# uclanlp/visualbert

Measured on NVIDIA H100. Metric: image-text pairs/sec fwd+bwd VisualBERT-base, higher is better.
Workload: dtype bf16

## Files before the change

### visualbert_b200/csrc/vb_api.cu

```cuda
#include <string.h>

#include "vb_internal.h"

namespace vb {

constexpr float kLnEps = 1e-12f;
constexpr unsigned kEmbedDropStream = 0xE0000001u;
enum { kSiteAttnProbs = 0, kSiteAttnOut = 1, kSiteFfnOut = 2 };
static inline unsigned drop_stream(unsigned layer, unsigned site) { return layer * 8u + site; }

#define VB_TRY(expr)            \
    do {                        \
        int _rc = (expr);       \
        if (_rc) return _rc;    \
    } while (0)

static vb_gemm_args fwd_args(const void* A, const void* W, void* D, int M, int N, int K) {
    vb_gemm_args a;
    memset(&a, 0, sizeof(a));
    a.A = A; a.lda = K; a.B = W; a.ldb = K; a.M = M; a.N = N; a.K = K; a.D = D; a.ldd = N;
    return a;
}
static vb_gemm_args dgrad_args(const void* dY, const void* W, void* dX, int M, int N, int K) {
    vb_gemm_args a;
    memset(&a, 0, sizeof(a));
    a.A = dY; a.lda = N; a.B = W; a.ldb = K; a.b_mn_major = 1; a.M = M; a.N = K; a.K = N; a.D = dX; a.ldd = K;
    return a;
}
static vb_gemm_args wgrad_args(const void* dY, const void* X, float* dW, int M, int N, int K) {
    vb_gemm_args a;
    memset(&a, 0, sizeof(a));
    a.A = dY; a.lda = N; a.a_mn_major = 1; a.B = X; a.ldb = K; a.b_mn_major = 1;
    a.M = N; a.N = K; a.K = M; a.D = dW; a.ldd = K; a.d_fp32 = 1;
    return a;
}

struct LayerRows {
    const int* cu_seqlens;
    int total;
};
static const LayerRows kDenseRows = {nullptr, 0};

static int check_layer(const vb_layer_desc* d, const LayerRows& r) {
    VB_REQUIRE(d != nullptr, "layer: null descriptor");
    VB_REQUIRE(d->batch > 0 && d->seq > 0, "layer: empty batch");
    VB_REQUIRE(d->hidden == d->heads * 64, "layer: hidden (%d) must equal heads (%d) * 64", d->hidden, d->heads);
    VB_REQUIRE(d->hidden % 16 == 0 && d->inter % 16 == 0, "layer: hidden/intermediate must be multiples of 16");
    VB_REQUIRE(d->w_qkv && d->w_attn_out && d->w_inter && d->w_out, "layer: null weight pointer");
    VB_REQUIRE(r.cu_seqlens != nullptr || d->mask_bias != nullptr, "layer: null mask_bias");
    VB_REQUIRE(r.cu_seqlens == nullptr || r.total > 0, "layer: varlen call without rows (total = %d)", r.total);
    return 0;
}

int layer_fwd(const vb_layer_desc* d, const void* x_in, void* x_out, const vb_layer_acts* s, cudaStream_t st,
              const LayerRows& rows = kDenseRows, bool for_bwd = true) {
    VB_TRY(check_layer(d, rows));
    VB_REQUIRE(x_in && x_out && s, "layer_fwd: null pointer");
    const bool vl = rows.cu_seqlens != nullptr;
    const int M = vl ? rows.total : d->batch * d->seq, H = d->hidden, I = d->inter;
    vb_gemm_args a = fwd_args(x_in, d->w_qkv, s->qkv, M, 3 * H, H);
    a.bias = d->b_qkv;
    VB_TRY(gemm(a, st));
    if (vl)
        VB_TRY(attn_fwd_varlen(s->qkv, rows.cu_seqlens, s->ctx, s->lse, s->keep_mask, d->batch, d->seq, rows.total, d->heads, H,
                               d->attn_dropout, d->seed, drop_stream(d->layer_index, kSiteAttnProbs), st, for_bwd));
    else
        VB_TRY(attn_fwd(s->qkv, d->mask_bias, s->ctx, s->lse, s->keep_mask, d->batch, d->seq, d->heads, H, d->attn_dropout, d->seed,
                        drop_stream(d->layer_index, kSiteAttnProbs), st));
    a = fwd_args(s->ctx, d->w_attn_out, s->pre1, M, H, H);
    a.bias = d->b_attn_out; a.addend = x_in; a.ld_add = H;
    a.dropout_p = d->hidden_dropout; a.dropout_seed = d->seed; a.dropout_stream = drop_stream(d->layer_index, kSiteAttnOut);
    VB_TRY(gemm(a, st));
    VB_TRY(ln_fwd(s->pre1, H, d->ln1_gamma, d->ln1_beta, s->x1, H, s->mean1, s->rstd1, M, H, kLnEps, st));
    if (for_bwd) {
        a = fwd_args(s->x1, d->w_inter, s->u, M, I, H);
        a.bias = d->b_inter; a.epilogue = VB_EPI_GELU; a.aux_out = s->g; a.ld_aux = I;
        a.gp_tiled = gemm_gp_tiled_ok(M, I) ? 1 : 0;
    } else {
        a = fwd_args(s->x1, d->w_inter, s->g, M, I, H);
        a.bias = d->b_inter; a.epilogue = VB_EPI_GELU_FWD;
    }
    VB_TRY(gemm(a, st));
    a = fwd_args(s->g, d->w_out, s->pre2, M, H, I);
    a.bias = d->b_out; a.addend = s->x1; a.ld_add = H;
    a.dropout_p = d->hidden_dropout; a.dropout_seed = d->seed; a.dropout_stream = drop_stream(d->layer_index, kSiteFfnOut);
    VB_TRY(gemm(a, st));
    VB_TRY(ln_fwd(s->pre2, H, d->ln2_gamma, d->ln2_beta, x_out, H, s->mean2, s->rstd2, M, H, kLnEps, st));
    return 0;
}

static long long layer_bwd_det_bytes(int M, int H, int I) {
    const long long c = colsum_det_bytes(M, I) > colsum_det_bytes(M, 3 * H) ? colsum_det_bytes(M, I) : colsum_det_bytes(M, 3 * H);
    return ln_bwd_det_bytes(M, H) > c ? ln_bwd_det_bytes(M, H) : c;
}

int layer_bwd(const vb_layer_desc* d, const void* x_in, const vb_layer_acts* s, const void* dy, void* dx,
              const vb_layer_grads* g, const vb_layer_scratch* w, cudaStream_t st, const LayerRows& rows = kDenseRows) {
    VB_TRY(check_layer(d, rows));
    VB_REQUIRE(x_in && s && dy && dx && g && w, "layer_bwd: null pointer");
    const bool vl = rows.cu_seqlens != nullptr;
    const int M = vl ? rows.total : d->batch * d->seq, H = d->hidden, I = d->inter;
    VB_TRY(det_require(layer_bwd_det_bytes(M, H, I), "layer backward"));
    const bool hd = d->hidden_dropout > 0.f;
    VB_REQUIRE(!hd || w->d_pre_drop, "layer_bwd: d_pre_drop scratch required when hidden_dropout > 0");
    void* dpm = hd ? w->d_pre_drop : w->d_pre;

    VB_TRY(ln_bwd(dy, s->pre2, s->mean2, s->rstd2, d->ln2_gamma, w->d_pre, hd ? w->d_pre_drop : nullptr, g->dln2_gamma,
                  g->dln2_beta, g->db_out, M, H, d->hidden_dropout, d->seed, drop_stream(d->layer_index, kSiteFfnOut),
                  0.f, 0, st));
    VB_TRY(gemm(wgrad_args(dpm, s->g, g->dw_out, M, H, I), st));
    vb_gemm_args a = dgrad_args(dpm, d->w_out, w->d_big, M, H, I);
    a.epilogue = VB_EPI_DGELU; a.aux_in = s->u; a.ld_aux = I;
    a.gp_tiled = gemm_gp_tiled_ok(M, I) ? 1 : 0;
    VB_TRY(gemm(a, st));
    VB_TRY(colsum(w->d_big, I, g->db_inter, M, I, st));
    VB_TRY(gemm(wgrad_args(w->d_big, s->x1, g->dw_inter, M, I, H), st));
    a = dgrad_args(w->d_big, d->w_inter, w->d_x1, M, I, H);
    a.addend = w->d_pre; a.ld_add = H;
    VB_TRY(gemm(a, st));
    VB_TRY(ln_bwd(w->d_x1, s->pre1, s->mean1, s->rstd1, d->ln1_gamma, w->d_pre, hd ? w->d_pre_drop : nullptr,
                  g->dln1_gamma, g->dln1_beta, g->db_attn_out, M, H, d->hidden_dropout, d->seed,
                  drop_stream(d->layer_index, kSiteAttnOut), 0.f, 0, st));
    VB_TRY(gemm(wgrad_args(dpm, s->ctx, g->dw_attn_out, M, H, H), st));
    a = dgrad_args(dpm, d->w_attn_out, w->d_ctx, M, H, H);
    const bool fused_delta = gemm_delta_ok(M, H) && w->drow != nullptr && attn_route(d->seq) != AttnRoute::Staged;
    if (fused_delta) { a.delta_ctx = s->ctx; a.delta_out = w->drow; a.delta_seq = vl ? rows.total : d->seq; }
    VB_TRY(gemm(a, st));
    if (vl)
        VB_TRY(attn_bwd_varlen(s->qkv, rows.cu_seqlens, s->ctx, s->lse, s->keep_mask, w->d_ctx, w->d_big, w->drow, d->batch, d->seq,
                               rows.total, d->heads, H, d->attn_dropout, d->seed, drop_stream(d->layer_index, kSiteAttnProbs), st,
                               fused_delta));
    else
        VB_TRY(attn_bwd(s->qkv, d->mask_bias, s->ctx, s->lse, s->keep_mask, w->d_ctx, w->d_big, w->drow, d->batch, d->seq, d->heads, H,
                        d->attn_dropout, d->seed, drop_stream(d->layer_index, kSiteAttnProbs), st, fused_delta));
    VB_TRY(colsum(w->d_big, 3 * H, g->db_qkv, M, 3 * H, st));
    VB_TRY(gemm(wgrad_args(w->d_big, x_in, g->dw_qkv, M, 3 * H, H), st));
    a = dgrad_args(w->d_big, d->w_qkv, dx, M, 3 * H, H);
    a.addend = w->d_pre; a.ld_add = H;
    VB_TRY(gemm(a, st));
    return 0;
}

static long long align256(long long x) { return (x + 255) / 256 * 256; }

long long encoder_arena_layout(int B, int S, int H, int A, int I, int attn_drop, long long* off, long long packed_rows = -1) {
    const long long M = packed_rows >= 0 ? packed_rows : static_cast<long long>(B) * S;
    const long long sizes[VB_ENCODER_ARENA_BUFFERS] = {
        M * 3 * H * 2, M * H * 2, static_cast<long long>(A) * M * 4, M * H * 2, M * 4, M * 4, M * H * 2, M * I * 2, M * I * 2,
        M * H * 2, M * 4, M * 4, attn_drop ? attn_keep_bytes(B, S, A) : 0, M * H * 2};
    long long o = 0;
    for (int i = 0; i < VB_ENCODER_ARENA_BUFFERS; ++i) {
        if (off) off[i] = o;
        o += align256(sizes[i]);
    }
    return o;
}

static void arena_acts(const vb_layer_desc* d, void* arena, int l, vb_layer_acts* a, void** y, const LayerRows& rows) {
    long long off[VB_ENCODER_ARENA_BUFFERS];
    const long long stride = encoder_arena_layout(d->batch, d->seq, d->hidden, d->heads, d->inter, d->attn_dropout > 0.f, off,
                                                  rows.cu_seqlens != nullptr ? rows.total : -1);
    char* base = static_cast<char*>(arena) + l * stride;
    a->qkv = base + off[0]; a->ctx = base + off[1]; a->lse = reinterpret_cast<float*>(base + off[2]);
    a->pre1 = base + off[3]; a->mean1 = reinterpret_cast<float*>(base + off[4]); a->rstd1 = reinterpret_cast<float*>(base + off[5]);
    a->x1 = base + off[6]; a->u = base + off[7]; a->g = base + off[8]; a->pre2 = base + off[9];
    a->mean2 = reinterpret_cast<float*>(base + off[10]); a->rstd2 = reinterpret_cast<float*>(base + off[11]);
    a->keep_mask = d->attn_dropout > 0.f ? base + off[12] : nullptr;
    *y = base + off[13];
}

int encoder_fwd(const vb_layer_desc* descs, int n, const void* x_in, void* arena, cudaStream_t st, const LayerRows& rows = kDenseRows) {
    VB_REQUIRE(descs && n > 0 && x_in && arena, "encoder_fwd: null pointer / no layers");
    const void* x = x_in;
    for (int l = 0; l < n; ++l) {
        VB_REQUIRE(descs[l].batch == descs[0].batch && descs[l].seq == descs[0].seq && descs[l].hidden == descs[0].hidden &&
                   descs[l].heads == descs[0].heads && descs[l].inter == descs[0].inter &&
                   (descs[l].attn_dropout > 0.f) == (descs[0].attn_dropout > 0.f), "encoder_fwd: layers differ in shape");
        vb_layer_acts a;
        void* y;
        arena_acts(&descs[l], arena, l, &a, &y, rows);
        VB_TRY(layer_fwd(&descs[l], x, y, &a, st, rows));
        x = y;
    }
    return 0;
}

int encoder_bwd(const vb_layer_desc* descs, int n, const void* x_in, void* arena, const void* dy, void* dx,
                const vb_layer_grads* grads, const vb_layer_scratch* w, cudaStream_t st, const LayerRows& rows = kDenseRows) {
    VB_REQUIRE(descs && n > 0 && x_in && arena && dy && dx && grads && w, "encoder_bwd: null pointer / no layers");
    const void* g_in = dy;
    for (int l = n - 1; l >= 0; --l) {
        vb_layer_acts a;
        void* y;
        arena_acts(&descs[l], arena, l, &a, &y, rows);
        const void* xl = x_in;
        if (l > 0) {
            vb_layer_acts ap;
            void* yp;
            arena_acts(&descs[l - 1], arena, l - 1, &ap, &yp, rows);
            xl = yp;
        }
        VB_TRY(layer_bwd(&descs[l], xl, &a, g_in, dx, &grads[l], w, st, rows));
        g_in = dx;
    }
    return 0;
}

enum { kWsQkv, kWsCtx, kWsPre, kWsX1, kWsG, kWsKeep, kWsY0, kWsY1, kWsBuffers };

long long infer_workspace_layout(int B, int S, int H, int A, int I, int attn_drop, long long packed_rows, long long* off) {
    const long long M = packed_rows >= 0 ? packed_rows : static_cast<long long>(B) * S;
    const long long sizes[kWsBuffers] = {M * 3 * H * 2, M * H * 2, M * H * 2, M * H * 2, M * I * 2,
                                         attn_drop ? attn_keep_bytes(B, S, A) : 0, M * H * 2, M * H * 2};
    long long o = 0;
    for (int i = 0; i < kWsBuffers; ++i) {
        if (off) off[i] = o;
        o += align256(sizes[i]);
    }
    return o;
}

int encoder_infer(const vb_layer_desc* descs, int n, const void* x_in, void* workspace, void* y_last, void* y_all, float* probs,
                  cudaStream_t st, const LayerRows& rows = kDenseRows) {
    VB_REQUIRE(descs && n > 0, "encoder_infer: null descriptors / no layers");
    VB_REQUIRE(x_in && workspace, "encoder_infer: null x_in / workspace");
    VB_REQUIRE(y_last || y_all, "encoder_infer: y_last and y_all are both NULL");
    const vb_layer_desc& d0 = descs[0];
    for (int l = 0; l < n; ++l) {
        VB_TRY(check_layer(&descs[l], rows));
        VB_REQUIRE(descs[l].batch == d0.batch && descs[l].seq == d0.seq && descs[l].hidden == d0.hidden && descs[l].heads == d0.heads &&
                   descs[l].inter == d0.inter && (descs[l].attn_dropout > 0.f) == (d0.attn_dropout > 0.f),
                   "encoder_infer: layers differ in shape");
    }
    const bool vl = rows.cu_seqlens != nullptr;
    const long long M = vl ? rows.total : static_cast<long long>(d0.batch) * d0.seq;
    const long long y_bytes = M * d0.hidden * 2;
    char* const ya = static_cast<char*>(y_all);
    VB_REQUIRE(!ya || !y_last || y_last == ya + (n - 1) * y_bytes, "encoder_infer: with y_all, y_last must be NULL or its last slice");
    long long off[kWsBuffers];
    infer_workspace_layout(d0.batch, d0.seq, d0.hidden, d0.heads, d0.inter, d0.attn_dropout > 0.f, vl ? rows.total : -1, off);
    char* const ws = static_cast<char*>(workspace);
    vb_layer_acts a;
    memset(&a, 0, sizeof(a));
    a.qkv = ws + off[kWsQkv]; a.ctx = ws + off[kWsCtx]; a.pre1 = a.pre2 = ws + off[kWsPre]; a.x1 = ws + off[kWsX1]; a.g = ws + off[kWsG];
    a.keep_mask = d0.attn_dropout > 0.f ? ws + off[kWsKeep] : nullptr;
    const long long per_layer = static_cast<long long>(d0.batch) * d0.heads * d0.seq * d0.seq;
    const void* x = x_in;
    for (int l = 0; l < n; ++l) {
        void* y = ya ? ya + l * y_bytes : l == n - 1 ? y_last : ws + off[(l & 1) ? kWsY1 : kWsY0];
        VB_TRY(layer_fwd(&descs[l], x, y, &a, st, rows, false));
        if (probs)
            VB_TRY(attn_probs(a.qkv, descs[l].mask_bias, probs + l * per_layer, d0.batch, d0.seq, d0.heads, d0.hidden, st));
        x = y;
    }
    return 0;
}

int encoder_attention_probs(const vb_layer_desc* descs, int n, void* arena, float* probs, cudaStream_t st) {
    VB_REQUIRE(descs && n > 0 && arena && probs, "encoder_attention_probs: null pointer / no layers");
    for (int l = 0; l < n; ++l) {
        VB_TRY(check_layer(&descs[l], kDenseRows));
        VB_REQUIRE(descs[l].batch == descs[0].batch && descs[l].seq == descs[0].seq && descs[l].hidden == descs[0].hidden &&
                   descs[l].heads == descs[0].heads && descs[l].inter == descs[0].inter &&
                   (descs[l].attn_dropout > 0.f) == (descs[0].attn_dropout > 0.f), "encoder_attention_probs: layers differ in shape");
    }
    const long long per_layer = static_cast<long long>(descs[0].batch) * descs[0].heads * descs[0].seq * descs[0].seq;
    for (int l = 0; l < n; ++l) {
        vb_layer_acts a;
        void* y;
        arena_acts(&descs[l], arena, l, &a, &y, kDenseRows);
        VB_TRY(attn_probs(a.qkv, descs[l].mask_bias, probs + l * per_layer, descs[l].batch, descs[l].seq, descs[l].heads,
                          descs[l].hidden, st));
    }
    return 0;
}

static int check_embed(const vb_embed_desc* d) {
    VB_REQUIRE(d != nullptr, "embed: null descriptor");
    VB_REQUIRE(d->batch > 0 && d->text_len > 0 && d->num_regions >= 0, "embed: bad shape");
    VB_REQUIRE(d->hidden % 16 == 0, "embed: hidden must be a multiple of 16");
    VB_REQUIRE(d->num_regions == 0 || (d->visual_dim % 8 == 0 && d->visual_feats && d->w_proj && d->visual_type),
               "embed: visual inputs missing or visual_dim not a multiple of 8");
    return 0;
}

int embed_fwd_api(const vb_embed_desc* d, void* y, const vb_embed_acts* s, cudaStream_t st) {
    VB_TRY(check_embed(d));
    VB_REQUIRE(y && s && s->pre && s->mean && s->rstd, "embed_fwd: null pointer");
    VB_REQUIRE(all_aligned16(d->word, d->pos, d->type, d->pos_vis, d->type_vis, s->pre, s->vis_proj, y),
               "embed_fwd: the fp32 tables, pre, vis_proj and y must be 16-byte aligned");
    const int BV = d->batch * d->num_regions;
    if (BV > 0) {
        vb_gemm_args a = fwd_args(d->visual_feats, d->w_proj, s->vis_proj, BV, d->hidden, d->visual_dim);
        a.bias = d->b_proj;
        if (d->visual_addend != nullptr) {
            a.addend = d->visual_addend;
            a.ld_add = d->hidden;
        }
        VB_TRY(gemm(a, st));
    }
    EmbedParams p;
    memset(&p, 0, sizeof(p));
    p.ids = reinterpret_cast<const long long*>(d->input_ids);
    p.tt = reinterpret_cast<const long long*>(d->token_type_ids);
    p.vt = reinterpret_cast<const long long*>(d->visual_type);
    p.vis_proj = static_cast<const bf16*>(s->vis_proj);
    p.word = d->word; p.pos = d->pos; p.type = d->type; p.pos_vis = d->pos_vis; p.type_vis = d->type_vis;
    p.gamma = d->gamma; p.beta = d->beta;
    p.pre = static_cast<bf16*>(s->pre); p.y = static_cast<bf16*>(y); p.mean = s->mean; p.rstd = s->rstd;
    p.B = d->batch; p.T = d->text_len; p.V = d->num_regions; p.H = d->hidden;
    p.vocab = d->vocab; p.max_pos = d->max_pos; p.n_types = d->n_types;
    p.eps = d->eps;
    if (d->dropout > 0.f) {
        const DropQ q = dropout_quantise(d->dropout);
        p.drop_scale = q.scale;
        p.drop_thresh16 = q.thr8;
        p.drop_seed = d->seed;
        p.drop_stream = kEmbedDropStream;
        p.drop_offset = drop_offset();
    }
    return embed_fwd(p, st);
}

int embed_bwd_api(const vb_embed_desc* d, const vb_embed_acts* s, const void* dy, const vb_embed_grads* g,
                  cudaStream_t st) {
    VB_TRY(check_embed(d));
    VB_REQUIRE(s && dy && g && g->d_pre, "embed_bwd: null pointer");
    VB_REQUIRE(all_aligned16(g->dword, g->dpos, g->d_vis), "embed_bwd: dword, dpos and d_vis must be 16-byte aligned");
    const int M = d->batch * (d->text_len + d->num_regions), H = d->hidden, BV = d->batch * d->num_regions;
    if (det_ws().ptr != nullptr) {
        const long long temp = embed_sort_temp_bytes(d->batch, d->text_len, d->num_regions);
        VB_REQUIRE(temp >= 0, "embed_bwd: radix sort size query failed");
        long long need = embed_bwd_det_bytes(d->batch, d->text_len, d->num_regions, H, temp);
        if (ln_bwd_det_bytes(M, H) > need) need = ln_bwd_det_bytes(M, H);
        if (BV > 0 && colsum_det_bytes(BV, H) > need) need = colsum_det_bytes(BV, H);
        VB_TRY(det_require(need, "embed_bwd"));
    }
    VB_TRY(ln_bwd(dy, s->pre, s->mean, s->rstd, d->gamma, g->d_pre, nullptr, g->dgamma, g->dbeta, nullptr, M, H, 0.f,
                  d->seed, 0, d->dropout, kEmbedDropStream, st));
    EmbedBwdParams p;
    memset(&p, 0, sizeof(p));
    p.de = static_cast<const bf16*>(g->d_pre);
    p.ids = reinterpret_cast<const long long*>(d->input_ids);
    p.tt = reinterpret_cast<const long long*>(d->token_type_ids);
    p.vt = reinterpret_cast<const long long*>(d->visual_type);
    p.dword = g->dword; p.dpos = g->dpos; p.dtype = g->dtype; p.dpos_vis = g->dpos_vis; p.dtype_vis = g->dtype_vis;
    p.dvis = static_cast<bf16*>(g->d_vis);
    p.B = d->batch; p.T = d->text_len; p.V = d->num_regions; p.H = H;
    p.vocab = d->vocab; p.max_pos = d->max_pos; p.n_types = d->n_types;
    VB_TRY(embed_bwd(p, st));
    if (BV > 0) {
        VB_TRY(colsum(g->d_vis, H, g->db_proj, BV, H, st));
        VB_TRY(gemm(wgrad_args(g->d_vis, d->visual_feats, g->dw_proj, BV, H, d->visual_dim), st));
        if (g->d_feats) VB_TRY(gemm(dgrad_args(g->d_vis, d->w_proj, g->d_feats, BV, H, d->visual_dim), st));
    }
    return 0;
}

static int max_splits(long long tiles, int rows) {
    int splits = 1;
    for (int kb = 1; kb <= gemm_k_blocks(rows); ++kb) { const int s = wgrad_splits(tiles, kb); if (s > splits) splits = s; }
    return splits;
}
long long deterministic_workspace_bytes(long long rows, int H, int I, int vocab, int adam_chunks) {
    long long need = 4LL * adam_chunks;
    auto up = [&](long long b) { if (b > need) need = b; };
    if (rows > 0 && H > 0) {
        const int R = rows < (1LL << 30) ? static_cast<int>(rows) : (1 << 30);
        auto colsum_bound = [&](long long N) { return 4 * (N > 6LL * 256 * num_sms() ? N : 6LL * 256 * num_sms()); };
        const int shapes[4][2] = {{3 * H, H}, {H, H}, {I, H}, {H, I}};
        for (const auto& sh : shapes) {
            if (sh[0] <= 0 || sh[1] <= 0) continue;
            const int splits = max_splits(gemm_tiles(sh[0], sh[1]), R);
            if (splits > 1) up(static_cast<long long>(splits) * sh[0] * sh[1] * 4);
        }
        long long last_tiles = -1;
        int splits = 1;
        for (int v = 16; v <= (vocab + 15) / 16 * 16; v += 16) {
            const long long t = gemm_tiles(v, H);
            if (t != last_tiles) { splits = max_splits(t, R); last_tiles = t; }
            if (splits > 1) up(static_cast<long long>(splits) * v * H * 4);
        }
        up(colsum_bound((vocab + 15) / 16 * 16));
        up(colsum_bound(I > 3 * H ? I : 3 * H));
        up(ln_bwd_det_bytes(R, H));
        up(embed_bwd_det_bytes(1, R, 0, H, -1));
    }
    return align256(need);
}

}

extern "C" {
int64_t vb_deterministic_workspace_bytes(int64_t rows, int32_t hidden, int32_t inter, int32_t vocab, int32_t adam_chunks) {
    if (rows < 0 || hidden < 0 || inter < 0 || vocab < 0 || adam_chunks < 0 || (rows > 0 && hidden % 8 != 0)) {
        vb::set_error("vb_deterministic_workspace_bytes: bad shape (rows %lld, hidden %d, inter %d, vocab %d, adam_chunks %d)",
                      static_cast<long long>(rows), hidden, inter, vocab, adam_chunks);
        return -1;
    }
    return vb::deterministic_workspace_bytes(rows, hidden, inter, vocab, adam_chunks);
}
int vb_layer_fwd(const vb_layer_desc* d, const void* x_in, void* x_out, const vb_layer_acts* acts, void* stream) {
    return vb::layer_fwd(d, x_in, x_out, acts, static_cast<cudaStream_t>(stream));
}
int vb_layer_bwd(const vb_layer_desc* d, const void* x_in, const vb_layer_acts* acts, const void* dy, void* dx,
                 const vb_layer_grads* grads, const vb_layer_scratch* scratch, void* stream) {
    return vb::layer_bwd(d, x_in, acts, dy, dx, grads, scratch, static_cast<cudaStream_t>(stream));
}
int64_t vb_encoder_arena_layout(int32_t batch, int32_t seq, int32_t hidden, int32_t heads, int32_t inter, int32_t attn_dropout_on,
                                int64_t* offsets) {
    long long off[VB_ENCODER_ARENA_BUFFERS];
    const long long stride = vb::encoder_arena_layout(batch, seq, hidden, heads, inter, attn_dropout_on, off);
    if (offsets) for (int i = 0; i < VB_ENCODER_ARENA_BUFFERS; ++i) offsets[i] = off[i];
    return stride;
}
int vb_encoder_fwd(const vb_layer_desc* descs, int32_t n_layers, const void* x_in, void* arena, void* stream) {
    return vb::encoder_fwd(descs, n_layers, x_in, arena, static_cast<cudaStream_t>(stream));
}
int vb_encoder_bwd(const vb_layer_desc* descs, int32_t n_layers, const void* x_in, void* arena, const void* dy, void* dx,
                   const vb_layer_grads* grads, const vb_layer_scratch* scratch, void* stream) {
    return vb::encoder_bwd(descs, n_layers, x_in, arena, dy, dx, grads, scratch, static_cast<cudaStream_t>(stream));
}
int vb_encoder_attention_probs(const vb_layer_desc* descs, int32_t n_layers, void* arena, float* probs, void* stream) {
    return vb::encoder_attention_probs(descs, n_layers, arena, probs, static_cast<cudaStream_t>(stream));
}
int64_t vb_encoder_arena_layout_varlen(int32_t batch, int32_t max_seq, int32_t total, int32_t hidden, int32_t heads, int32_t inter,
                                       int32_t attn_dropout_on, int64_t* offsets) {
    if (batch <= 0 || max_seq <= 0 || total < 0) {
        vb::set_error("vb_encoder_arena_layout_varlen: bad shape (batch %d, max_seq %d, total %d)", batch, max_seq, total);
        return -1;
    }
    long long off[VB_ENCODER_ARENA_BUFFERS];
    const long long stride = vb::encoder_arena_layout(batch, max_seq, hidden, heads, inter, attn_dropout_on, off, total);
    if (offsets) for (int i = 0; i < VB_ENCODER_ARENA_BUFFERS; ++i) offsets[i] = off[i];
    return stride;
}
int vb_encoder_fwd_varlen(const vb_layer_desc* descs, int32_t n_layers, const int32_t* cu_seqlens, int32_t total, const void* x_in,
                          void* arena, void* stream) {
    if (cu_seqlens == nullptr) { vb::set_error("vb_encoder_fwd_varlen: cu_seqlens is NULL"); return 2; }
    if (total <= 0) { vb::set_error("vb_encoder_fwd_varlen: total (%d) must be > 0", total); return 2; }
    const vb::LayerRows rows = {cu_seqlens, total};
    return vb::encoder_fwd(descs, n_layers, x_in, arena, static_cast<cudaStream_t>(stream), rows);
}
int64_t vb_encoder_infer_workspace(int32_t batch, int32_t seq, int32_t hidden, int32_t heads, int32_t inter, int32_t attn_dropout_on,
                                   int64_t packed_rows) {
    if (batch <= 0 || seq <= 0 || hidden <= 0 || heads <= 0 || inter <= 0 || packed_rows == 0 || packed_rows >= (1LL << 31)) {
        vb::set_error("vb_encoder_infer_workspace: bad shape (batch %d, seq %d, hidden %d, heads %d, inter %d, packed_rows %lld)", batch,
                      seq, hidden, heads, inter, static_cast<long long>(packed_rows));
        return -1;
    }
    return vb::infer_workspace_layout(batch, seq, hidden, heads, inter, attn_dropout_on, packed_rows, nullptr);
}
int vb_encoder_infer(const vb_layer_desc* descs, int32_t n_layers, const void* x_in, void* workspace, void* y_last, void* y_all,
                     float* probs, void* stream) {
    return vb::encoder_infer(descs, n_layers, x_in, workspace, y_last, y_all, probs, static_cast<cudaStream_t>(stream));
}
int vb_encoder_infer_varlen(const vb_layer_desc* descs, int32_t n_layers, const int32_t* cu_seqlens, int32_t total, const void* x_in,
                            void* workspace, void* y_last, void* y_all, void* stream) {
    if (cu_seqlens == nullptr) { vb::set_error("vb_encoder_infer_varlen: cu_seqlens is NULL"); return 2; }
    if (total <= 0) { vb::set_error("vb_encoder_infer_varlen: total (%d) must be > 0", total); return 2; }
    const vb::LayerRows rows = {cu_seqlens, total};
    return vb::encoder_infer(descs, n_layers, x_in, workspace, y_last, y_all, nullptr, static_cast<cudaStream_t>(stream), rows);
}
int vb_encoder_bwd_varlen(const vb_layer_desc* descs, int32_t n_layers, const int32_t* cu_seqlens, int32_t total, const void* x_in,
                          void* arena, const void* dy, void* dx, const vb_layer_grads* grads, const vb_layer_scratch* scratch,
                          void* stream) {
    if (cu_seqlens == nullptr) { vb::set_error("vb_encoder_bwd_varlen: cu_seqlens is NULL"); return 2; }
    if (total <= 0) { vb::set_error("vb_encoder_bwd_varlen: total (%d) must be > 0", total); return 2; }
    const vb::LayerRows rows = {cu_seqlens, total};
    return vb::encoder_bwd(descs, n_layers, x_in, arena, dy, dx, grads, scratch, static_cast<cudaStream_t>(stream), rows);
}
int vb_embed_fwd(const vb_embed_desc* d, void* y, const vb_embed_acts* acts, void* stream) {
    return vb::embed_fwd_api(d, y, acts, static_cast<cudaStream_t>(stream));
}
int vb_embed_bwd(const vb_embed_desc* d, const vb_embed_acts* acts, const void* dy, const vb_embed_grads* g, void* stream) {
    return vb::embed_bwd_api(d, acts, dy, g, static_cast<cudaStream_t>(stream));
}
int vb_mask_bias(const int64_t* input_mask, const int64_t* image_mask, float* out, int32_t batch, int32_t text_len,
                 int32_t num_regions, void* stream) {
    return vb::mask_bias(reinterpret_cast<const long long*>(input_mask), reinterpret_cast<const long long*>(image_mask),
                         out, batch, text_len, num_regions, static_cast<cudaStream_t>(stream));
}
int vb_cast_f32_to_bf16(const float* src, void* dst, int64_t n, void* stream) {
    return vb::cast_f32_bf16(src, dst, n, static_cast<cudaStream_t>(stream));
}
int vb_cast_bf16_to_f32(const void* src, float* dst, int64_t n, void* stream) {
    return vb::cast_bf16_f32(src, dst, n, static_cast<cudaStream_t>(stream));
}
int vb_colsum_bf16(const void* x, int64_t ld, float* out, int32_t rows, int32_t cols, void* stream) {
    return vb::colsum(x, ld, out, rows, cols, static_cast<cudaStream_t>(stream));
}
}
```

### visualbert_b200/csrc/vb_attention.cu

```cuda
#include "vb_attention.cuh"
#include "vb_internal.h"

namespace vb {


template <int MT, bool VL, bool OFF>
__device__ __forceinline__ void attn_fwd_body(const AttnParams& p, const int nsub, const unsigned long long* drop_offset = nullptr,
                                              unsigned long long seed64 = 0, unsigned stream_id = 0) {
    constexpr int NT = 128 / MT;
    extern __shared__ __align__(128) uint8_t dsmem[];
    __shared__ float sbias[kMaxSub * kBlk];
    const int tid = threadIdx.x, warp = tid >> 5, lane = tid & 31;
    const int g = lane >> 2, t = lane & 3;
    const int qb = blockIdx.x, h = blockIdx.y, b = blockIdx.z;
    const SeqSpan sp = seq_span<VL>(p, b, h);
    const int S = sp.len;
    if (VL && qb * kBlk >= S) return;
    const long long ld = 3LL * p.H;
    const bf16* qbase = p.qkv + sp.row0 * ld + h * kHd;
    const bf16* kbase = qbase + p.H;
    const bf16* vbase = qbase + 2 * p.H;
    const uint32_t sQ = smem_u32(dsmem), sK0 = sQ + kTileBytes, sV0 = sK0 + nsub * kTileBytes;
    const int nkb = (p.S + kBlk - 1) / kBlk;
    const int nkv = VL ? (S + kBlk - 1) / kBlk : nkb;

    const float sc2 = p.scale * kLog2e;
    float m[MT][2], l[MT][2];
    float o[MT][8][4];
#pragma unroll
    for (int mt = 0; mt < MT; ++mt) {
        m[mt][0] = m[mt][1] = -INFINITY;
        l[mt][0] = l[mt][1] = 0.f;
        zero_acc(o[mt]);
    }
    uint32_t qf[MT][4][4];
    const unsigned bh = static_cast<unsigned>(b * p.A + h);
    const int qrow0 = qb * kBlk + warp * 16 * MT;
    const bool active = qrow0 < S;

    for (int kb0 = 0; kb0 < nkv; kb0 += nsub) {
        const int nb = min(nsub, nkv - kb0);
        if (kb0 > 0) __syncthreads();
        if (kb0 == 0) load_tile<NT>(sQ, qbase, ld, qb * kBlk, S, tid);
        for (int j = 0; j < nb; ++j) {
            load_tile<NT>(sK0 + j * kTileBytes, kbase, ld, (kb0 + j) * kBlk, S, tid);
            load_tile<NT>(sV0 + j * kTileBytes, vbase, ld, (kb0 + j) * kBlk, S, tid);
            cp_async_commit();
        }
        for (int i = tid; i < nb * kBlk; i += NT) {
            const int key = kb0 * kBlk + i;
            sbias[i] = key_bias2<VL>(p, b, key, S);
        }
        for (int j = 0; j < nb; ++j) {
            cp_async_wait_dyn(nb - 1 - j);
            __syncthreads();
            if (!active) continue;
            if (kb0 == 0 && j == 0) {
#pragma unroll
                for (int mt = 0; mt < MT; ++mt) load_afrag(qf[mt], sQ, warp * 16 * MT + mt * 16, lane);
            }
            const int kb = kb0 + j;
            const int kvalid = min(kBlk, S - kb * kBlk);
            float s[MT][8][4];
#pragma unroll
            for (int mt = 0; mt < MT; ++mt) zero_acc(s[mt]);
            gemm_nt_mt<MT>(s, qf, sK0 + j * kTileBytes, lane, kvalid);
            uint32_t pf[MT][4][4];
#pragma unroll
            for (int mt = 0; mt < MT; ++mt) {
                float mx[2] = {-INFINITY, -INFINITY};
#pragma unroll
                for (int nt = 0; nt < 8; ++nt) {
                    const float b0 = sbias[j * kBlk + nt * 8 + 2 * t], b1 = sbias[j * kBlk + nt * 8 + 2 * t + 1];
                    s[mt][nt][0] = fmaf(s[mt][nt][0], sc2, b0); s[mt][nt][1] = fmaf(s[mt][nt][1], sc2, b1);
                    s[mt][nt][2] = fmaf(s[mt][nt][2], sc2, b0); s[mt][nt][3] = fmaf(s[mt][nt][3], sc2, b1);
                    mx[0] = fmaxf(mx[0], fmaxf(s[mt][nt][0], s[mt][nt][1]));
                    mx[1] = fmaxf(mx[1], fmaxf(s[mt][nt][2], s[mt][nt][3]));
                }
                float alpha[2];
#pragma unroll
                for (int r = 0; r < 2; ++r) {
                    mx[r] = fmaxf(mx[r], __shfl_xor_sync(0xffffffffu, mx[r], 1));
                    mx[r] = fmaxf(mx[r], __shfl_xor_sync(0xffffffffu, mx[r], 2));
                    const float mn = fmaxf(m[mt][r], mx[r]);
                    alpha[r] = fast_ex2(m[mt][r] - mn);
                    m[mt][r] = mn;
                }
                float rs[2] = {0.f, 0.f};
#pragma unroll
                for (int nt = 0; nt < 8; ++nt) {
                    s[mt][nt][0] = fast_ex2(s[mt][nt][0] - m[mt][0]); s[mt][nt][1] = fast_ex2(s[mt][nt][1] - m[mt][0]);
                    s[mt][nt][2] = fast_ex2(s[mt][nt][2] - m[mt][1]); s[mt][nt][3] = fast_ex2(s[mt][nt][3] - m[mt][1]);
                    rs[0] += s[mt][nt][0] + s[mt][nt][1];
                    rs[1] += s[mt][nt][2] + s[mt][nt][3];
                }
#pragma unroll
                for (int r = 0; r < 2; ++r) {
                    rs[r] += __shfl_xor_sync(0xffffffffu, rs[r], 1);
                    rs[r] += __shfl_xor_sync(0xffffffffu, rs[r], 2);
                    l[mt][r] = l[mt][r] * alpha[r] + rs[r];
                }
#pragma unroll
                for (int nt = 0; nt < 8; ++nt) {
                    o[mt][nt][0] *= alpha[0]; o[mt][nt][1] *= alpha[0];
                    o[mt][nt][2] *= alpha[1]; o[mt][nt][3] *= alpha[1];
                }
                if (p.drop_scale != 0.f) {
                    const int qa = qrow0 + mt * 16 + g, qc = qa + 8;
                    const unsigned sd = OFF ? attn_seed_fold(seed64 + *drop_offset, stream_id) : p.drop_seed;
                    const uint32_t ka_bits = attn_keep16(sd, bh, qa, kb, t, nkb, p.drop_thresh16);
                    const uint32_t kc_bits = attn_keep16(sd, bh, qc, kb, t, nkb, p.drop_thresh16);
#pragma unroll
                    for (int nt = 0; nt < 8; ++nt) {
                        s[mt][nt][0] = ((ka_bits >> (2 * nt)) & 1u) ? s[mt][nt][0] * p.drop_scale : 0.f;
                        s[mt][nt][1] = ((ka_bits >> (2 * nt + 1)) & 1u) ? s[mt][nt][1] * p.drop_scale : 0.f;
                        s[mt][nt][2] = ((kc_bits >> (2 * nt)) & 1u) ? s[mt][nt][2] * p.drop_scale : 0.f;
                        s[mt][nt][3] = ((kc_bits >> (2 * nt + 1)) & 1u) ? s[mt][nt][3] * p.drop_scale : 0.f;
                    }
                    const unsigned long long ma = quad_mask64(ka_bits, t), mc = quad_mask64(kc_bits, t);
                    if (t == 0) {
                        unsigned long long* kp = p.keep + (static_cast<unsigned long long>(bh) * (nkb * kBlk)) * nkb;
                        kp[static_cast<long long>(qa) * nkb + kb] = ma;
                        kp[static_cast<long long>(qc) * nkb + kb] = mc;
                    }
                }
                acc_to_afrag(pf[mt], s[mt]);
            }
            gemm_nn_mt<MT>(o, pf, sV0 + j * kTileBytes, lane, kvalid);
        }
    }
    if (!active) return;
#pragma unroll
    for (int mt = 0; mt < MT; ++mt) {
        const int r0 = qrow0 + mt * 16;
        const float inv0 = 1.f / l[mt][0], inv1 = 1.f / l[mt][1];
        store_acc(p.ctx + sp.row0 * p.H + h * kHd, p.H, r0, S, o[mt], lane, inv0, inv1);
        if (t == 0 && p.lse != nullptr) {
            float* lse = p.lse + sp.stat0;
            if (r0 + g < S) lse[r0 + g] = (m[mt][0] + log2f(l[mt][0])) * 0.6931471805599453f;
            if (r0 + g + 8 < S) lse[r0 + g + 8] = (m[mt][1] + log2f(l[mt][1])) * 0.6931471805599453f;
        }
    }
}

template <int MT, int MINB, bool VL = false>
__global__ void __launch_bounds__(128 / MT, MINB) attn_fwd_kernel(const AttnParams p, const int nsub) { attn_fwd_body<MT, VL, false>(p, nsub); }
template <int MT, int MINB, bool VL = false>
__global__ void __launch_bounds__(128 / MT, MINB)
attn_fwd_off_kernel(const AttnParams p, const int nsub, const unsigned long long* drop_offset, unsigned long long seed64, unsigned stream_id) {
    attn_fwd_body<MT, VL, true>(p, nsub, drop_offset, seed64, stream_id);
}

template <int MINB, bool VL = false>
__global__ void __launch_bounds__(128, MINB)
attn_bwd_dq_kernel(const AttnParams p, const int nsub) {
    extern __shared__ __align__(128) uint8_t dsmem[];
    __shared__ float sbias[kMaxSub * kBlk];
    __shared__ float sD[kBlk];
    const int tid = threadIdx.x, warp = tid >> 5, lane = tid & 31;
    const int g = lane >> 2, t = lane & 3;
    const int qb = blockIdx.x, h = blockIdx.y, b = blockIdx.z;
    const SeqSpan sp = seq_span<VL>(p, b, h);
    const int S = sp.len;
    if (VL && qb * kBlk >= S) return;
    const long long ld = 3LL * p.H;
    const bf16* qbase = p.qkv + sp.row0 * ld + h * kHd;
    const bf16* kbase = qbase + p.H;
    const bf16* vbase = qbase + 2 * p.H;
    const bf16* obase = p.ctx + sp.row0 * p.H + h * kHd;
    const bf16* dobase = p.dctx + sp.row0 * p.H + h * kHd;
    const uint32_t sQ = smem_u32(dsmem), sdO = sQ + kTileBytes, sO = sQ + 2 * kTileBytes;
    const uint32_t sK0 = sQ + 3 * kTileBytes, sV0 = sK0 + nsub * kTileBytes;
    const int nkb = (p.S + kBlk - 1) / kBlk;
    const int nkv = VL ? (S + kBlk - 1) / kBlk : nkb;
    const int qrow0 = qb * kBlk + warp * 16;
    const bool active = qrow0 < S;
    const float* lsep = p.lse + sp.stat0;
    const float lse0 = (qrow0 + g < S) ? lsep[qrow0 + g] * kLog2e : 0.f;
    const float lse1 = (qrow0 + g + 8 < S) ? lsep[qrow0 + g + 8] * kLog2e : 0.f;
    const float sc2 = p.scale * kLog2e;
    const unsigned bh = static_cast<unsigned>(b * p.A + h);
    uint32_t qf[4][4], dof[4][4];
    float d0 = 0.f, d1 = 0.f;
    float dq[8][4];
    zero_acc(dq);

    for (int kb0 = 0; kb0 < nkv; kb0 += nsub) {
        const int nb = min(nsub, nkv - kb0);
        if (kb0 > 0) __syncthreads();
        if (kb0 == 0) {
            load_tile(sQ, qbase, ld, qb * kBlk, S, tid);
            load_tile(sdO, dobase, p.H, qb * kBlk, S, tid);
            load_tile(sO, obase, p.H, qb * kBlk, S, tid);
        }
        for (int j = 0; j < nb; ++j) {
            load_tile(sK0 + j * kTileBytes, kbase, ld, (kb0 + j) * kBlk, S, tid);
            load_tile(sV0 + j * kTileBytes, vbase, ld, (kb0 + j) * kBlk, S, tid);
            cp_async_commit();
        }
        for (int i = tid; i < nb * kBlk; i += 128) {
            const int key = kb0 * kBlk + i;
            sbias[i] = key_bias2<VL>(p, b, key, S);
        }
        for (int j = 0; j < nb; ++j) {
            cp_async_wait_dyn(nb - 1 - j);
            __syncthreads();
            if (kb0 == 0 && j == 0) {
                const int r = tid >> 1, half = tid & 1;
                float acc = 0.f;
#pragma unroll
                for (int c = 0; c < 4; ++c) {
                    const int chunk = half * 4 + c;
                    const uint4 a = *reinterpret_cast<const uint4*>(dsmem + kTileBytes + swz(r, chunk));
                    const uint4 ov = *reinterpret_cast<const uint4*>(dsmem + 2 * kTileBytes + swz(r, chunk));
                    const uint32_t av[4] = {a.x, a.y, a.z, a.w}, bv[4] = {ov.x, ov.y, ov.z, ov.w};
#pragma unroll
                    for (int i = 0; i < 4; ++i) {
                        const float2 x = unpack_bf16x2(av[i]), y = unpack_bf16x2(bv[i]);
                        acc += x.x * y.x + x.y * y.y;
                    }
                }
                acc += __shfl_xor_sync(0xffffffffu, acc, 1);
                if (half == 0) {
                    sD[r] = acc;
                    const int q = qb * kBlk + r;
                    if (q < S) p.drow[sp.stat0 + q] = acc;
                }
                __syncthreads();
                if (active) {
                    load_afrag(qf, sQ, warp * 16, lane);
                    load_afrag(dof, sdO, warp * 16, lane);
                    d0 = sD[warp * 16 + g];
                    d1 = sD[warp * 16 + g + 8];
                }
            }
            if (!active) continue;
            const int kb = kb0 + j;
            const int kvalid = min(kBlk, S - kb * kBlk);
            float s[8][4];
            zero_acc(s);
            unsigned long long keep_a = 0, keep_c = 0;
            if (p.drop_scale != 0.f) {
                const unsigned long long* kp = p.keep + (static_cast<unsigned long long>(bh) * (nkb * kBlk)) * nkb;
                keep_a = kp[static_cast<long long>(qrow0 + g) * nkb + kb];
                keep_c = kp[static_cast<long long>(qrow0 + g + 8) * nkb + kb];
            }
            gemm_nt(s, qf, sK0 + j * kTileBytes, lane, kvalid);
#pragma unroll
            for (int hh = 0; hh < 2; ++hh) {
                float dp[4][4];
#pragma unroll
                for (int i = 0; i < 4; ++i) dp[i][0] = dp[i][1] = dp[i][2] = dp[i][3] = 0.f;
                gemm_nt_half(dp, dof, sV0 + j * kTileBytes, lane, hh, kvalid);
#pragma unroll
                for (int n4 = 0; n4 < 4; ++n4) {
                    const int nt = hh * 4 + n4;
                    const float b0 = sbias[j * kBlk + nt * 8 + 2 * t], b1 = sbias[j * kBlk + nt * 8 + 2 * t + 1];
                    const float p0 = fast_ex2(fmaf(s[nt][0], sc2, b0) - lse0), p1 = fast_ex2(fmaf(s[nt][1], sc2, b1) - lse0);
                    const float p2 = fast_ex2(fmaf(s[nt][2], sc2, b0) - lse1), p3 = fast_ex2(fmaf(s[nt][3], sc2, b1) - lse1);
                    float e0 = dp[n4][0], e1 = dp[n4][1], e2 = dp[n4][2], e3 = dp[n4][3];
                    if (p.drop_scale != 0.f) {
                        const int bit = nt * 8 + 2 * t;
                        e0 = ((keep_a >> bit) & 1ull) ? e0 * p.drop_scale : 0.f;
                        e1 = ((keep_a >> (bit + 1)) & 1ull) ? e1 * p.drop_scale : 0.f;
                        e2 = ((keep_c >> bit) & 1ull) ? e2 * p.drop_scale : 0.f;
                        e3 = ((keep_c >> (bit + 1)) & 1ull) ? e3 * p.drop_scale : 0.f;
                    }
                    s[nt][0] = p0 * (e0 - d0); s[nt][1] = p1 * (e1 - d0);
                    s[nt][2] = p2 * (e2 - d1); s[nt][3] = p3 * (e3 - d1);
                }
            }
            uint32_t dsf[4][4];
            acc_to_afrag(dsf, s);
            gemm_nn(dq, dsf, sK0 + j * kTileBytes, lane, kvalid);
        }
    }
    if (!active) return;
    store_acc(p.dqkv + sp.row0 * ld + h * kHd, ld, qrow0, S, dq, lane, p.scale, p.scale);
}

template <int MINB, bool VL = false>
__global__ void __launch_bounds__(128, MINB)
attn_bwd_dkv_kernel(const AttnParams p, const int nsub) {
    extern __shared__ __align__(128) uint8_t dsmem[];
    __shared__ float slse[kMaxSub * kBlk];
    __shared__ float sD[kMaxSub * kBlk];
    const int tid = threadIdx.x, warp = tid >> 5, lane = tid & 31;
    const int g = lane >> 2, t = lane & 3;
    const int kbk = blockIdx.x, h = blockIdx.y, b = blockIdx.z;
    const SeqSpan sp = seq_span<VL>(p, b, h);
    const int S = sp.len;
    if (VL && kbk * kBlk >= S) return;
    const long long ld = 3LL * p.H;
    const bf16* qbase = p.qkv + sp.row0 * ld + h * kHd;
    const bf16* kbase = qbase + p.H;
    const bf16* vbase = qbase + 2 * p.H;
    const bf16* dobase = p.dctx + sp.row0 * p.H + h * kHd;
    const uint32_t sK = smem_u32(dsmem), sV = sK + kTileBytes, sQ0 = sK + 2 * kTileBytes, sdO0 = sQ0 + nsub * kTileBytes;
    const int nqb = (p.S + kBlk - 1) / kBlk;
    const int nqv = VL ? (S + kBlk - 1) / kBlk : nqb;
    const float* lsep = p.lse + sp.stat0;
    const float* drp = p.drow + sp.stat0;
    const int krow0 = kbk * kBlk + warp * 16;
    const bool active = krow0 < S;
    const int ka = krow0 + g, kc = krow0 + g + 8;
    const float bias0 = key_bias2<VL>(p, b, ka, S);
    const float bias1 = key_bias2<VL>(p, b, kc, S);
    const float sc2 = p.scale * kLog2e;
    const unsigned bh = static_cast<unsigned>(b * p.A + h);
    float dk[8][4], dv[8][4];
    zero_acc(dk);
    zero_acc(dv);

    for (int qb0 = 0; qb0 < nqv; qb0 += nsub) {
        const int nb = min(nsub, nqv - qb0);
        if (qb0 > 0) __syncthreads();
        if (qb0 == 0) {
            load_tile(sK, kbase, ld, kbk * kBlk, S, tid);
            load_tile(sV, vbase, ld, kbk * kBlk, S, tid);
        }
        for (int j = 0; j < nb; ++j) {
            load_tile(sQ0 + j * kTileBytes, qbase, ld, (qb0 + j) * kBlk, S, tid);
            load_tile(sdO0 + j * kTileBytes, dobase, p.H, (qb0 + j) * kBlk, S, tid);
            cp_async_commit();
        }
        for (int i = tid; i < nb * kBlk; i += 128) {
            const int q = qb0 * kBlk + i;
            slse[i] = q < S ? lsep[q] * kLog2e : INFINITY;
            sD[i] = q < S ? drp[q] : 0.f;
        }
        for (int j = 0; j < nb; ++j) {
            cp_async_wait_dyn(nb - 1 - j);
            __syncthreads();
            if (!active) continue;
            const int qb = qb0 + j;
            const int qvalid = min(kBlk, S - qb * kBlk);
            uint32_t af[4][4];
            float st[8][4];
            zero_acc(st);
            load_afrag(af, sK, warp * 16, lane);
            gemm_nt(st, af, sQ0 + j * kTileBytes, lane, qvalid);
#pragma unroll
            for (int nt = 0; nt < 8; ++nt) {
                const int qi = nt * 8 + 2 * t;
                const float l0 = slse[j * kBlk + qi], l1 = slse[j * kBlk + qi + 1];
                st[nt][0] = fast_ex2(fmaf(st[nt][0], sc2, bias0) - l0); st[nt][1] = fast_ex2(fmaf(st[nt][1], sc2, bias0) - l1);
                st[nt][2] = fast_ex2(fmaf(st[nt][2], sc2, bias1) - l0); st[nt][3] = fast_ex2(fmaf(st[nt][3], sc2, bias1) - l1);
            }
            unsigned keepbits = 0xffffffffu;
            if (p.drop_scale != 0.f) {
                keepbits = 0;
#pragma unroll
                const unsigned short* kp16 = reinterpret_cast<const unsigned short*>(
                    p.keep + (static_cast<unsigned long long>(bh) * (nqb * kBlk)) * nqb) + kbk * 4 + warp;
#pragma unroll
                for (int nt = 0; nt < 8; ++nt) {
                    const long long q = qb * kBlk + nt * 8 + 2 * t;
                    const unsigned w0 = kp16[q * (nqb * 4)], w1 = kp16[(q + 1) * (nqb * 4)];
                    keepbits |= ((w0 >> g) & 1u) << (nt * 4);
                    keepbits |= ((w1 >> g) & 1u) << (nt * 4 + 1);
                    keepbits |= ((w0 >> (8 + g)) & 1u) << (nt * 4 + 2);
                    keepbits |= ((w1 >> (8 + g)) & 1u) << (nt * 4 + 3);
                }
            }
            const float ds = p.drop_scale != 0.f ? p.drop_scale : 1.f;
#pragma unroll
            for (int jj = 0; jj < 4; ++jj) {
                float w[8];
#pragma unroll
                for (int e = 0; e < 8; ++e) {
                    const int nt = 2 * jj + (e >> 2), c = e & 3;
                    w[e] = ((keepbits >> (nt * 4 + c)) & 1u) ? st[nt][c] * ds : 0.f;
                }
                af[jj][0] = pack_bf16x2(w[0], w[1]); af[jj][1] = pack_bf16x2(w[2], w[3]);
                af[jj][2] = pack_bf16x2(w[4], w[5]); af[jj][3] = pack_bf16x2(w[6], w[7]);
            }
            gemm_nn(dv, af, sdO0 + j * kTileBytes, lane, qvalid);
            load_afrag(af, sV, warp * 16, lane);
#pragma unroll
            for (int hh = 0; hh < 2; ++hh) {
                float dpt[4][4];
#pragma unroll
                for (int i = 0; i < 4; ++i) dpt[i][0] = dpt[i][1] = dpt[i][2] = dpt[i][3] = 0.f;
                gemm_nt_half(dpt, af, sdO0 + j * kTileBytes, lane, hh, qvalid);
#pragma unroll
                for (int n4 = 0; n4 < 4; ++n4) {
                    const int nt = hh * 4 + n4;
                    const int qi = nt * 8 + 2 * t;
                    const float dd0 = sD[j * kBlk + qi], dd1 = sD[j * kBlk + qi + 1];
#pragma unroll
                    for (int c = 0; c < 4; ++c) {
                        const float e = ((keepbits >> (nt * 4 + c)) & 1u) ? dpt[n4][c] * ds : 0.f;
                        st[nt][c] *= e - ((c & 1) ? dd1 : dd0);
                    }
                }
            }
            acc_to_afrag(af, st);
            gemm_nn(dk, af, sQ0 + j * kTileBytes, lane, qvalid);
        }
    }
    if (!active) return;
    bf16* dbase = p.dqkv + sp.row0 * ld + h * kHd;
    store_acc(dbase + p.H, ld, krow0, S, dk, lane, p.scale, p.scale);
    store_acc(dbase + 2 * p.H, ld, krow0, S, dv, lane, 1.f, 1.f);
}

static bool aligned16(const void* ptr) { return (reinterpret_cast<uintptr_t>(ptr) & 15) == 0; }

static int fill_params(AttnParams& p, const void* qkv, const float* mask_bias, void* ctx, float* lse,
                       const void* dctx, void* dqkv, float* drow, void* keep, int B, int S, int A, int H,
                       float dropout_p, unsigned long long seed, unsigned stream_id, AttnDropOffset* off = nullptr) {
    VB_REQUIRE(B > 0 && S > 0 && A > 0, "attention: empty problem");
    VB_REQUIRE(H == A * kHd, "attention: head_dim must be 64 (hidden=%d heads=%d)", H, A);
    VB_REQUIRE(A <= 65535 && B <= 65535, "attention: grid too large");
    VB_REQUIRE(dropout_p >= 0.f && dropout_p < 1.f, "attention: dropout_p out of range");
    VB_REQUIRE(dropout_p == 0.f || keep != nullptr, "attention: dropout needs the keep-mask buffer (vb_attention_keep_bytes)");
    VB_REQUIRE(aligned16(qkv) && (dctx == nullptr || (aligned16(ctx) && aligned16(dctx))),
               "attention: qkv, ctx (backward) and dctx must be 16-byte aligned");
    p.keep = static_cast<unsigned long long*>(keep);
    p.qkv = static_cast<const bf16*>(qkv);
    p.mask_bias = mask_bias;
    p.ctx = static_cast<bf16*>(ctx);
    p.lse = lse;
    p.dctx = static_cast<const bf16*>(dctx);
    p.dqkv = static_cast<bf16*>(dqkv);
    p.drow = drow;
    p.B = B; p.S = S; p.A = A; p.H = H;
    p.cu_seqlens = nullptr;
    p.total = 0;
    p.scale = 0.125f;
    const unsigned th8 = static_cast<unsigned>(dropout_p * 256.f + 0.5f);
    p.drop_thresh16 = th8;
    p.drop_scale = dropout_p > 0.f ? 256.f / (256.f - static_cast<float>(th8 > 255 ? 255 : th8)) : 0.f;
    p.drop_seed = attn_seed_fold(seed, stream_id);
    if (off != nullptr) *off = AttnDropOffset{dropout_p > 0.f ? drop_offset() : nullptr, seed, stream_id};
    return 0;
}

long long attn_keep_bytes(int B, int S, int A) {
    const long long nkb = (S + kBlk - 1) / kBlk;
    return 2 * static_cast<long long>(B) * A * (nkb * kBlk) * nkb * 8;
}

static int set_varlen(AttnParams& p, const int* cu_seqlens, int total, const void* qkv, const void* out) {
    VB_REQUIRE(cu_seqlens != nullptr, "attention varlen: cu_seqlens is NULL");
    VB_REQUIRE(total >= 0, "attention varlen: total (%d) must be >= 0", total);
    VB_REQUIRE(qkv != nullptr && out != nullptr, "attention varlen: null pointer");
    VB_REQUIRE(static_cast<long long>(p.A) * total < (1LL << 31), "attention varlen: heads * total too large");
    p.cu_seqlens = cu_seqlens;
    p.total = total;
    return 0;
}

static int attn_fwd_launch(const AttnParams& p, const AttnDropOffset& off, cudaStream_t st) {
    const int B = p.B, S = p.S, A = p.A;
    dim3 grid((S + kBlk - 1) / kBlk, A, B);
    const AttnRoute route = attn_route(S);
    if (route == AttnRoute::Wgmma) return attn_fwd_wgmma(p, off, st);
    if (route == AttnRoute::Head) return attn_fwd_head(p, off, static_cast<int>(grid.x), st);
    const long long nkb = grid.x;
    VB_REQUIRE(p.drop_scale == 0.f || static_cast<long long>(B) * A * (nkb * kBlk) * nkb * 16 < (1LL << 32),
               "attention dropout: mask counter space exceeded (B*A*S too large)");
    const int nsub = static_cast<int>(grid.x) < kMaxSub ? static_cast<int>(grid.x) : kMaxSub;
    const int smem = (1 + 2 * nsub) * kTileBytes;
    static int configured[kMaxDevices] = {0}, configured_vl[kMaxDevices] = {0};
    static int configured_off[kMaxDevices] = {0}, configured_vl_off[kMaxDevices] = {0};
    {
        ProfScope ps(st, PROF_ATTN_FWD, 4.0 * B * A * S * S * kHd, 1);
        if (off.offset != nullptr && p.cu_seqlens == nullptr) {
            VB_CHECK_CUDA(ensure_dyn_smem(attn_fwd_off_kernel<1, 3>, (1 + 2 * kMaxSub) * kTileBytes, configured_off));
            attn_fwd_off_kernel<1, 3><<<grid, 128, smem, st>>>(p, nsub, off.offset, off.seed, off.stream_id);
        } else if (off.offset != nullptr) {
            VB_CHECK_CUDA(ensure_dyn_smem(attn_fwd_off_kernel<1, 3, true>, (1 + 2 * kMaxSub) * kTileBytes, configured_vl_off));
            attn_fwd_off_kernel<1, 3, true><<<grid, 128, smem, st>>>(p, nsub, off.offset, off.seed, off.stream_id);
        } else if (p.cu_seqlens == nullptr) {
            VB_CHECK_CUDA(ensure_dyn_smem(attn_fwd_kernel<1, 3>, (1 + 2 * kMaxSub) * kTileBytes, configured));
            attn_fwd_kernel<1, 3><<<grid, 128, smem, st>>>(p, nsub);
        } else {
            VB_CHECK_CUDA(ensure_dyn_smem(attn_fwd_kernel<1, 3, true>, (1 + 2 * kMaxSub) * kTileBytes, configured_vl));
            attn_fwd_kernel<1, 3, true><<<grid, 128, smem, st>>>(p, nsub);
        }
    }
    VB_CHECK_CUDA(cudaGetLastError());
    return 0;
}

int attn_fwd(const void* qkv, const float* mask_bias, void* ctx, float* lse, void* keep, int B, int S, int A, int H,
             float dropout_p, unsigned long long seed, unsigned stream_id, cudaStream_t st) {
    AttnParams p;
    AttnDropOffset off;
    int rc = fill_params(p, qkv, mask_bias, ctx, lse, nullptr, nullptr, nullptr, keep, B, S, A, H, dropout_p, seed, stream_id, &off);
    if (rc) return rc;
    return attn_fwd_launch(p, off, st);
}

int attn_fwd_varlen(const void* qkv, const int* cu_seqlens, void* ctx, float* lse, void* keep, int B, int max_seq, int total,
                    int A, int H, float dropout_p, unsigned long long seed, unsigned stream_id, cudaStream_t st, bool need_lse) {
    AttnParams p;
    AttnDropOffset off;
    int rc = fill_params(p, qkv, nullptr, ctx, lse, nullptr, nullptr, nullptr, keep, B, max_seq, A, H, dropout_p, seed, stream_id, &off);
    if (rc) return rc;
    VB_REQUIRE(lse != nullptr || !need_lse, "attention varlen: lse is NULL");
    if ((rc = set_varlen(p, cu_seqlens, total, qkv, ctx))) return rc;
    if (total == 0) return 0;
    return attn_fwd_launch(p, off, st);
}

static int attn_bwd_launch(const AttnParams& p, cudaStream_t st, bool delta_ready) {
    const int B = p.B, S = p.S, A = p.A;
    dim3 grid((S + kBlk - 1) / kBlk, A, B);
    const AttnRoute route = attn_route(S);
    if (route == AttnRoute::Wgmma) return attn_bwd_wgmma(p, st, delta_ready);
    if (route == AttnRoute::Head) return attn_bwd_head(p, static_cast<int>(grid.x), st, delta_ready);
    const int nsub = static_cast<int>(grid.x) < kMaxSub ? static_cast<int>(grid.x) : kMaxSub;
    const bool vl = p.cu_seqlens != nullptr;
    static int c0[kMaxDevices] = {0}, c1[kMaxDevices] = {0}, v0[kMaxDevices] = {0}, v1[kMaxDevices] = {0};
    if (vl) {
        VB_CHECK_CUDA(ensure_dyn_smem(attn_bwd_dq_kernel<3, true>, (3 + 2 * kMaxSub) * kTileBytes, v0));
        VB_CHECK_CUDA(ensure_dyn_smem(attn_bwd_dkv_kernel<3, true>, (2 + 2 * kMaxSub) * kTileBytes, v1));
    } else {
        VB_CHECK_CUDA(ensure_dyn_smem(attn_bwd_dq_kernel<3>, (3 + 2 * kMaxSub) * kTileBytes, c0));
        VB_CHECK_CUDA(ensure_dyn_smem(attn_bwd_dkv_kernel<3>, (2 + 2 * kMaxSub) * kTileBytes, c1));
    }
    {
        ProfScope ps(st, PROF_ATTN_DQ, 4.0 * B * A * S * S * kHd, 1);
        if (vl) attn_bwd_dq_kernel<3, true><<<grid, 128, (3 + 2 * nsub) * kTileBytes, st>>>(p, nsub);
        else attn_bwd_dq_kernel<3><<<grid, 128, (3 + 2 * nsub) * kTileBytes, st>>>(p, nsub);
    }
    {
        ProfScope ps(st, PROF_ATTN_DKV, 4.0 * B * A * S * S * kHd, 1);
        if (vl) attn_bwd_dkv_kernel<3, true><<<grid, 128, (2 + 2 * nsub) * kTileBytes, st>>>(p, nsub);
        else attn_bwd_dkv_kernel<3><<<grid, 128, (2 + 2 * nsub) * kTileBytes, st>>>(p, nsub);
    }
    VB_CHECK_CUDA(cudaGetLastError());
    return 0;
}

int attn_bwd(const void* qkv, const float* mask_bias, const void* ctx, const float* lse, const void* keep,
             const void* dctx, void* dqkv, float* drow, int B, int S, int A, int H, float dropout_p,
             unsigned long long seed, unsigned stream_id, cudaStream_t st, bool delta_ready) {
    AttnParams p;
    int rc = fill_params(p, qkv, mask_bias, const_cast<void*>(ctx), const_cast<float*>(lse), dctx, dqkv, drow,
                         const_cast<void*>(keep), B, S, A, H, dropout_p, seed, stream_id);
    if (rc) return rc;
    return attn_bwd_launch(p, st, delta_ready);
}

int attn_bwd_varlen(const void* qkv, const int* cu_seqlens, const void* ctx, const float* lse, const void* keep,
                    const void* dctx, void* dqkv, float* drow, int B, int max_seq, int total, int A, int H, float dropout_p,
                    unsigned long long seed, unsigned stream_id, cudaStream_t st, bool delta_ready) {
    AttnParams p;
    int rc = fill_params(p, qkv, nullptr, const_cast<void*>(ctx), const_cast<float*>(lse), dctx, dqkv, drow,
                         const_cast<void*>(keep), B, max_seq, A, H, dropout_p, seed, stream_id);
    if (rc) return rc;
    VB_REQUIRE(ctx && lse && dctx && drow, "attention varlen: null pointer");
    if ((rc = set_varlen(p, cu_seqlens, total, qkv, dqkv))) return rc;
    if (total == 0) return 0;
    return attn_bwd_launch(p, st, delta_ready);
}

}

extern "C" {
int64_t vb_attention_keep_bytes(int32_t batch, int32_t seq, int32_t heads) {
    return vb::attn_keep_bytes(batch, seq, heads);
}
int vb_attention_fwd(const void* qkv, const float* mask_bias, void* ctx, float* lse, void* keep_mask, int32_t batch,
                     int32_t seq, int32_t heads, int32_t hidden, float dropout_p, uint64_t dropout_seed,
                     uint32_t dropout_stream, void* stream) {
    return vb::attn_fwd(qkv, mask_bias, ctx, lse, keep_mask, batch, seq, heads, hidden, dropout_p, dropout_seed,
                        dropout_stream, static_cast<cudaStream_t>(stream));
}
int vb_attention_bwd(const void* qkv, const float* mask_bias, const void* ctx, const float* lse, const void* keep_mask,
                     const void* dctx, void* dqkv, float* drow, int32_t batch, int32_t seq, int32_t heads,
                     int32_t hidden, float dropout_p, uint64_t dropout_seed, uint32_t dropout_stream, void* stream) {
    return vb::attn_bwd(qkv, mask_bias, ctx, lse, keep_mask, dctx, dqkv, drow, batch, seq, heads, hidden, dropout_p,
                        dropout_seed, dropout_stream, static_cast<cudaStream_t>(stream), false);
}
int vb_attention_fwd_varlen(const void* qkv, const int32_t* cu_seqlens, void* ctx, float* lse, void* keep_mask, int32_t batch,
                            int32_t max_seq, int32_t total, int32_t heads, int32_t hidden, float dropout_p, uint64_t dropout_seed,
                            uint32_t dropout_stream, void* stream) {
    return vb::attn_fwd_varlen(qkv, cu_seqlens, ctx, lse, keep_mask, batch, max_seq, total, heads, hidden, dropout_p, dropout_seed,
                               dropout_stream, static_cast<cudaStream_t>(stream));
}
int vb_attention_bwd_varlen(const void* qkv, const int32_t* cu_seqlens, const void* ctx, const float* lse, const void* keep_mask,
                            const void* dctx, void* dqkv, float* drow, int32_t batch, int32_t max_seq, int32_t total, int32_t heads,
                            int32_t hidden, float dropout_p, uint64_t dropout_seed, uint32_t dropout_stream, void* stream) {
    return vb::attn_bwd_varlen(qkv, cu_seqlens, ctx, lse, keep_mask, dctx, dqkv, drow, batch, max_seq, total, heads, hidden,
                               dropout_p, dropout_seed, dropout_stream, static_cast<cudaStream_t>(stream), false);
}
}
```

### visualbert_b200/csrc/vb_attention.cuh

```cuda
#pragma once

#include "../../include/vbert_b200.h"
#include "vb_common.cuh"

namespace vb {


constexpr int kHd = 64;
constexpr int kBlk = 64;
constexpr int kTileBytes = kBlk * kHd * 2;
constexpr float kLog2e = 1.4426950408889634f;

struct AttnParams {
    const bf16* qkv;
    const float* mask_bias;
    bf16* ctx;
    float* lse;
    const bf16* dctx;
    bf16* dqkv;
    float* drow;
    unsigned long long* keep;
    int B, S, A, H;
    float scale;
    float drop_scale;
    unsigned drop_thresh16;
    unsigned drop_seed;
    const int* cu_seqlens;
    int total;
};

struct SeqSpan {
    long long row0;
    int len;
    long long stat0;
};
template <bool VL>
__device__ __forceinline__ SeqSpan seq_span(const AttnParams& p, int b, int h) {
    SeqSpan s;
    if constexpr (VL) {
        int lo = __ldg(p.cu_seqlens + b), hi = __ldg(p.cu_seqlens + b + 1);
        lo = min(max(lo, 0), p.total);
        hi = min(max(hi, lo), p.total);
        s.row0 = lo;
        s.len = min(hi - lo, p.S);
        s.stat0 = static_cast<long long>(h) * p.total + lo;
    } else {
        s.row0 = static_cast<long long>(b) * p.S;
        s.len = p.S;
        s.stat0 = (static_cast<long long>(b) * p.A + h) * p.S;
    }
    return s;
}
template <bool VL>
__device__ __forceinline__ float key_bias2(const AttnParams& p, int b, int key, int len) {
    if constexpr (VL) return key < len ? 0.f : -INFINITY;
    else return key < p.S ? p.mask_bias[static_cast<long long>(b) * p.S + key] * kLog2e : -INFINITY;
}

struct AttnDropOffset {
    const unsigned long long* offset;
    unsigned long long seed;
    unsigned stream_id;
};
__host__ __device__ __forceinline__ unsigned attn_seed_fold(unsigned long long seed, unsigned stream_id) {
    unsigned long long z = seed + 0x9E3779B97F4A7C15ull * (stream_id + 1ull);
    z = (z ^ (z >> 30)) * 0xBF58476D1CE4E5B9ull;
    z = (z ^ (z >> 27)) * 0x94D049BB133111EBull;
    return static_cast<unsigned>(z ^ (z >> 31));
}

__device__ __forceinline__ uint32_t swz(int row, int chunk) {
    return static_cast<uint32_t>(row * 128 + ((chunk ^ (row & 7)) << 4));
}
__device__ __forceinline__ void cp_async16(uint32_t dst, const void* src, bool valid) {
    const int sz = valid ? 16 : 0;
    asm volatile("cp.async.cg.shared.global [%0], [%1], 16, %2;" ::"r"(dst), "l"(src), "r"(sz) : "memory");
}
__device__ __forceinline__ void cp_async_commit() { asm volatile("cp.async.commit_group;" ::: "memory"); }
template <int N>
__device__ __forceinline__ void cp_async_wait() { asm volatile("cp.async.wait_group %0;" ::"n"(N) : "memory"); }

template <int NT = 128>
__device__ __forceinline__ void load_tile(uint32_t tile, const bf16* base, long long ld, int row0, int nrows,
                                          int tid) {
#pragma unroll
    for (int i = 0; i < 512 / NT; ++i) {
        const int idx = tid + i * NT;
        const int r = idx >> 3, c = idx & 7;
        const bool ok = (row0 + r) < nrows;
        const bf16* src = base + static_cast<long long>(ok ? row0 + r : 0) * ld + c * 8;
        cp_async16(tile + swz(r, c), src, ok);
    }
}

__device__ __forceinline__ void ldsm_x4(uint32_t addr, uint32_t& r0, uint32_t& r1, uint32_t& r2, uint32_t& r3) {
    asm volatile("ldmatrix.sync.aligned.m8n8.x4.shared.b16 {%0, %1, %2, %3}, [%4];"
                 : "=r"(r0), "=r"(r1), "=r"(r2), "=r"(r3) : "r"(addr));
}
__device__ __forceinline__ void st_shared_u32(uint32_t addr, uint32_t v) {
    asm volatile("st.shared.b32 [%0], %1;" ::"r"(addr), "r"(v) : "memory");
}
__device__ __forceinline__ void ldsm_x4_t(uint32_t addr, uint32_t& r0, uint32_t& r1, uint32_t& r2, uint32_t& r3) {
    asm volatile("ldmatrix.sync.aligned.m8n8.x4.trans.shared.b16 {%0, %1, %2, %3}, [%4];"
                 : "=r"(r0), "=r"(r1), "=r"(r2), "=r"(r3) : "r"(addr));
}
__device__ __forceinline__ void mma16816(float (&c)[4], const uint32_t (&a)[4], uint32_t b0, uint32_t b1) {
    asm volatile(
        "mma.sync.aligned.m16n8k16.row.col.f32.bf16.bf16.f32 {%0, %1, %2, %3}, {%4, %5, %6, %7}, {%8, %9}, "
        "{%0, %1, %2, %3};"
        : "+f"(c[0]), "+f"(c[1]), "+f"(c[2]), "+f"(c[3])
        : "r"(a[0]), "r"(a[1]), "r"(a[2]), "r"(a[3]), "r"(b0), "r"(b1));
}

__device__ __forceinline__ void load_afrag(uint32_t (&a)[4][4], uint32_t tile, int r0, int lane) {
    const int row = r0 + (lane & 7) + ((lane >> 3) & 1) * 8;
#pragma unroll
    for (int ks = 0; ks < 4; ++ks) {
        const int chunk = ks * 2 + (lane >> 4);
        ldsm_x4(tile + swz(row, chunk), a[ks][0], a[ks][1], a[ks][2], a[ks][3]);
    }
}
__device__ __forceinline__ void gemm_nt(float (&acc)[8][4], const uint32_t (&a)[4][4], uint32_t tile, int lane,
                                        int nvalid = 64) {
#pragma unroll
    for (int ks = 0; ks < 4; ++ks) {
#pragma unroll
        for (int np = 0; np < 4; ++np) {
            if (np * 16 < nvalid) {
                const int row = np * 16 + (lane & 7) + (lane >> 4) * 8;
                const int chunk = ks * 2 + ((lane >> 3) & 1);
                uint32_t b0, b1, b2, b3;
                ldsm_x4(tile + swz(row, chunk), b0, b1, b2, b3);
                mma16816(acc[2 * np], a[ks], b0, b1);
                mma16816(acc[2 * np + 1], a[ks], b2, b3);
            }
        }
    }
}
__device__ __forceinline__ void gemm_nn(float (&acc)[8][4], const uint32_t (&a)[4][4], uint32_t tile, int lane,
                                        int kvalid = 64) {
#pragma unroll
    for (int ks = 0; ks < 4; ++ks) {
        if (ks * 16 < kvalid) {
#pragma unroll
            for (int np = 0; np < 4; ++np) {
                const int row = ks * 16 + (lane & 7) + ((lane >> 3) & 1) * 8;
                const int chunk = np * 2 + (lane >> 4);
                uint32_t b0, b1, b2, b3;
                ldsm_x4_t(tile + swz(row, chunk), b0, b1, b2, b3);
                mma16816(acc[2 * np], a[ks], b0, b1);
                mma16816(acc[2 * np + 1], a[ks], b2, b3);
            }
        }
    }
}
template <int MT>
__device__ __forceinline__ void gemm_nt_mt(float (&acc)[MT][8][4], const uint32_t (&a)[MT][4][4], uint32_t tile, int lane,
                                           int nvalid) {
#pragma unroll
    for (int ks = 0; ks < 4; ++ks) {
#pragma unroll
        for (int np = 0; np < 4; ++np) {
            if (np * 16 < nvalid) {
                const int row = np * 16 + (lane & 7) + (lane >> 4) * 8;
                const int chunk = ks * 2 + ((lane >> 3) & 1);
                uint32_t b0, b1, b2, b3;
                ldsm_x4(tile + swz(row, chunk), b0, b1, b2, b3);
#pragma unroll
                for (int mt = 0; mt < MT; ++mt) {
                    mma16816(acc[mt][2 * np], a[mt][ks], b0, b1);
                    mma16816(acc[mt][2 * np + 1], a[mt][ks], b2, b3);
                }
            }
        }
    }
}
template <int MT>
__device__ __forceinline__ void gemm_nn_mt(float (&acc)[MT][8][4], const uint32_t (&a)[MT][4][4], uint32_t tile, int lane,
                                           int kvalid) {
#pragma unroll
    for (int ks = 0; ks < 4; ++ks) {
        if (ks * 16 < kvalid) {
#pragma unroll
            for (int np = 0; np < 4; ++np) {
                const int row = ks * 16 + (lane & 7) + ((lane >> 3) & 1) * 8;
                const int chunk = np * 2 + (lane >> 4);
                uint32_t b0, b1, b2, b3;
                ldsm_x4_t(tile + swz(row, chunk), b0, b1, b2, b3);
#pragma unroll
                for (int mt = 0; mt < MT; ++mt) {
                    mma16816(acc[mt][2 * np], a[mt][ks], b0, b1);
                    mma16816(acc[mt][2 * np + 1], a[mt][ks], b2, b3);
                }
            }
        }
    }
}
__device__ __forceinline__ void gemm_nt_half(float (&acc)[4][4], const uint32_t (&a)[4][4], uint32_t tile, int lane,
                                             int half, int nvalid) {
#pragma unroll
    for (int ks = 0; ks < 4; ++ks) {
#pragma unroll
        for (int q = 0; q < 2; ++q) {
            const int np = half * 2 + q;
            if (np * 16 < nvalid) {
                const int row = np * 16 + (lane & 7) + (lane >> 4) * 8;
                const int chunk = ks * 2 + ((lane >> 3) & 1);
                uint32_t b0, b1, b2, b3;
                ldsm_x4(tile + swz(row, chunk), b0, b1, b2, b3);
                mma16816(acc[2 * q], a[ks], b0, b1);
                mma16816(acc[2 * q + 1], a[ks], b2, b3);
            }
        }
    }
}
__device__ __forceinline__ void cp_async_wait_dyn(int pending) {
    switch (pending) {
        case 0: cp_async_wait<0>(); break;
        case 1: cp_async_wait<1>(); break;
        case 2: cp_async_wait<2>(); break;
        default: cp_async_wait<3>(); break;
    }
}
__device__ __forceinline__ void acc_to_afrag(uint32_t (&a)[4][4], const float (&p)[8][4]) {
#pragma unroll
    for (int j = 0; j < 4; ++j) {
        a[j][0] = pack_bf16x2(p[2 * j][0], p[2 * j][1]);
        a[j][1] = pack_bf16x2(p[2 * j][2], p[2 * j][3]);
        a[j][2] = pack_bf16x2(p[2 * j + 1][0], p[2 * j + 1][1]);
        a[j][3] = pack_bf16x2(p[2 * j + 1][2], p[2 * j + 1][3]);
    }
}
__device__ __forceinline__ void zero_acc(float (&c)[8][4]) {
#pragma unroll
    for (int i = 0; i < 8; ++i)
#pragma unroll
        for (int j = 0; j < 4; ++j) c[i][j] = 0.f;
}
__device__ __forceinline__ uint32_t attn_keep16(unsigned seed, unsigned bh, int q, int kb, int t, int nkb, unsigned thresh8) {
    const unsigned np64 = static_cast<unsigned>(nkb) * kBlk;
    const unsigned w = (bh * np64 + static_cast<unsigned>(q)) * static_cast<unsigned>(nkb) + static_cast<unsigned>(kb);
    const unsigned base = (w << 4) + (static_cast<unsigned>(t) << 2);
    uint32_t bits = 0;
#pragma unroll
    for (int j = 0; j < 4; ++j) {
        const uint32_t h = mix32((base + j) ^ seed);
        bits |= static_cast<uint32_t>((h & 0xffu) >= thresh8) << (4 * j);
        bits |= static_cast<uint32_t>(((h >> 8) & 0xffu) >= thresh8) << (4 * j + 1);
        bits |= static_cast<uint32_t>(((h >> 16) & 0xffu) >= thresh8) << (4 * j + 2);
        bits |= static_cast<uint32_t>((h >> 24) >= thresh8) << (4 * j + 3);
    }
    return bits;
}
__device__ __forceinline__ unsigned long long quad_mask64(uint32_t bits16, int t) {
    unsigned long long m = 0;
#pragma unroll
    for (int nt = 0; nt < 8; ++nt) m |= static_cast<unsigned long long>((bits16 >> (2 * nt)) & 3u) << (nt * 8 + 2 * t);
    m |= __shfl_xor_sync(0xffffffffu, m, 1);
    m |= __shfl_xor_sync(0xffffffffu, m, 2);
    return m;
}
__device__ __forceinline__ void store_acc(bf16* base, long long ld, int row0, int nrows, const float (&c)[8][4],
                                          int lane, float mul0, float mul1) {
    const int g = lane >> 2, t = lane & 3;
    const int ra = row0 + g, rb = row0 + g + 8;
#pragma unroll
    for (int nt = 0; nt < 8; ++nt) {
        const int col = nt * 8 + 2 * t;
        if (ra < nrows)
            *reinterpret_cast<uint32_t*>(base + static_cast<long long>(ra) * ld + col) =
                pack_bf16x2(c[nt][0] * mul0, c[nt][1] * mul0);
        if (rb < nrows)
            *reinterpret_cast<uint32_t*>(base + static_cast<long long>(rb) * ld + col) =
                pack_bf16x2(c[nt][2] * mul1, c[nt][3] * mul1);
    }
}


constexpr int kMaxSub = 4;

int attn_fwd_head(const AttnParams& p, const AttnDropOffset& off, int nkb, cudaStream_t st);
int attn_bwd_head(const AttnParams& p, int nkb, cudaStream_t st, bool delta_ready);
int attn_keep_mask(const AttnParams& p, const AttnDropOffset& off, int nkb, cudaStream_t st);
int attn_delta(const AttnParams& p, cudaStream_t st);
int attn_fwd_wgmma(const AttnParams& p, const AttnDropOffset& off, cudaStream_t st);
int attn_bwd_wgmma(const AttnParams& p, cudaStream_t st, bool delta_ready);
int make_tmap_bf16(CUtensorMap* m, const void* ptr, uint64_t inner, uint64_t outer, uint64_t ld_elems, uint32_t box_outer);

}
```

### visualbert_b200/csrc/vb_attention_wgmma.cu

```cuda
#include "vb_attention.cuh"

namespace vb {

constexpr int kWgTile = kBlk * kHd * 2;

template <int NKB>
struct AttnSmem {
    static constexpr int FWD_BYTES = 3 * NKB * kWgTile + NKB * kBlk * 4 + 16 + 1024;
    static constexpr int BWD_BYTES = (4 * NKB + NKB * NKB) * kWgTile + NKB * kBlk * 4 + 16 + 1024;
};

__device__ __forceinline__ uint64_t tile_desc(uint32_t saddr) { return wgmma_desc_sw128(saddr, kWgTile, 1024); }

__device__ __forceinline__ unsigned long long keep_word(const AttnParams& p, unsigned bh, int q, int kb, int nkb, int t) {
    if (p.drop_scale == 0.f) return ~0ull;
    return p.keep[(static_cast<unsigned long long>(bh) * (nkb * kBlk) + q) * nkb + kb] >> (2 * t);
}

template <int NKB>
__device__ __forceinline__ void qk_block(float (&s)[32], uint32_t sQ, uint32_t sK, int wg, int kb) {
#pragma unroll
    for (int k = 0; k < kHd / 16; ++k)
        wgmma_m64n64k16_ss<0, 0>(s, tile_desc(sQ + wg * kWgTile + k * 32), tile_desc(sK + kb * kWgTile + k * 32), k > 0 ? 1u : 0u);
}
__device__ __forceinline__ void pack_afrag(uint32_t (&a)[4], const float (&x)[32], int kk) {
    a[0] = pack_bf16x2(x[8 * kk], x[8 * kk + 1]);
    a[1] = pack_bf16x2(x[8 * kk + 2], x[8 * kk + 3]);
    a[2] = pack_bf16x2(x[8 * kk + 4], x[8 * kk + 5]);
    a[3] = pack_bf16x2(x[8 * kk + 6], x[8 * kk + 7]);
}
__device__ __forceinline__ void store_rows(bf16* base, long long ld, int r0, int nrows, const float (&x)[32], int t, float mul0, float mul1) {
#pragma unroll
    for (int j = 0; j < 8; ++j) {
        const int col = 8 * j + 2 * t;
        if (r0 < nrows) *reinterpret_cast<uint32_t*>(base + static_cast<long long>(r0) * ld + col) = pack_bf16x2(x[4 * j] * mul0, x[4 * j + 1] * mul0);
        if (r0 + 8 < nrows)
            *reinterpret_cast<uint32_t*>(base + static_cast<long long>(r0 + 8) * ld + col) = pack_bf16x2(x[4 * j + 2] * mul1, x[4 * j + 3] * mul1);
    }
}
__device__ __forceinline__ void store_tile(uint32_t tile, int r, const float (&x)[32], int t) {
#pragma unroll
    for (int j = 0; j < 8; ++j) {
        st_shared_u32(tile + swz(r, j) + 4 * t, pack_bf16x2(x[4 * j], x[4 * j + 1]));
        st_shared_u32(tile + swz(r + 8, j) + 4 * t, pack_bf16x2(x[4 * j + 2], x[4 * j + 3]));
    }
}

template <int NKB, bool VL = false>
__global__ void __launch_bounds__(NKB * 128, 1)
attn_fwd_wgmma_kernel(const __grid_constant__ CUtensorMap tmQKV, const AttnParams p) {
    extern __shared__ uint8_t smem_raw[];
    const uint32_t raw = smem_u32(smem_raw);
    const uint32_t base = (raw + 1023u) & ~1023u;
    uint8_t* smem = smem_raw + (base - raw);
    const uint32_t sQ = base, sK = base + NKB * kWgTile, sV = base + 2 * NKB * kWgTile;
    float* sbias = reinterpret_cast<float*>(smem + 3 * NKB * kWgTile);
    const uint32_t bar = base + 3 * NKB * kWgTile + NKB * kBlk * 4;
    const int tid = threadIdx.x, wg = tid >> 7, warp = (tid >> 5) & 3, lane = tid & 31, g = lane >> 2, t = lane & 3;
    const int item = blockIdx.x, b = item / p.A, h = item % p.A;
    const unsigned bh = static_cast<unsigned>(item);
    const SeqSpan sp = seq_span<VL>(p, b, h);
    const int S = sp.len;
    const int nkv = VL ? (S + kBlk - 1) / kBlk : NKB;
    const int row0 = VL ? static_cast<int>(sp.row0) : b * S;
    if (VL && S == 0) return;

    if (tid == 0) {
        tma_prefetch_desc(&tmQKV);
        mbar_init(bar, 1);
        fence_barrier_init();
    }
    __syncthreads();
    pdl_trigger();
    pdl_wait();
    if (tid == 0) {
        mbar_arrive_expect_tx(bar, 3 * nkv * kWgTile);
#pragma unroll
        for (int m = 0; m < 3; ++m)
#pragma unroll
            for (int kb = 0; kb < NKB; ++kb)
                if (!VL || kb < nkv) tma_load_2d(base + (m * NKB + kb) * kWgTile, &tmQKV, bar, m * p.H + h * kHd, row0 + kb * kBlk);
    }
    for (int i = tid; i < NKB * kBlk; i += NKB * 128) sbias[i] = key_bias2<VL>(p, b, i, S);
    const int q0 = wg * kBlk + warp * 16 + g;
    unsigned long long keep[NKB][2];
#pragma unroll
    for (int kb = 0; kb < NKB; ++kb) {
        keep[kb][0] = keep_word(p, bh, q0, kb, NKB, t);
        keep[kb][1] = keep_word(p, bh, q0 + 8, kb, NKB, t);
    }
    __syncthreads();
    if (VL && wg >= nkv) return;
    mbar_wait(bar, 0);

    float s[NKB][32];
    wgmma_fence();
#pragma unroll
    for (int kb = 0; kb < NKB; ++kb)
        if (!VL || kb < nkv) qk_block<NKB>(s[kb], sQ, sK, wg, kb);
    wgmma_commit();
    wgmma_wait<0>();

    const float sc2 = p.scale * kLog2e;
    float mx[2] = {-INFINITY, -INFINITY};
#pragma unroll
    for (int kb = 0; kb < NKB; ++kb)
#pragma unroll
        for (int j = 0; j < 8; ++j) {
            if (VL && kb >= nkv) break;
            const float b0 = sbias[kb * kBlk + 8 * j + 2 * t], b1 = sbias[kb * kBlk + 8 * j + 2 * t + 1];
            s[kb][4 * j] = fmaf(s[kb][4 * j], sc2, b0); s[kb][4 * j + 1] = fmaf(s[kb][4 * j + 1], sc2, b1);
            s[kb][4 * j + 2] = fmaf(s[kb][4 * j + 2], sc2, b0); s[kb][4 * j + 3] = fmaf(s[kb][4 * j + 3], sc2, b1);
            mx[0] = fmaxf(mx[0], fmaxf(s[kb][4 * j], s[kb][4 * j + 1]));
            mx[1] = fmaxf(mx[1], fmaxf(s[kb][4 * j + 2], s[kb][4 * j + 3]));
        }
    float l[2] = {0.f, 0.f};
#pragma unroll
    for (int r = 0; r < 2; ++r) {
        mx[r] = fmaxf(mx[r], __shfl_xor_sync(0xffffffffu, mx[r], 1));
        mx[r] = fmaxf(mx[r], __shfl_xor_sync(0xffffffffu, mx[r], 2));
    }
#pragma unroll
    for (int kb = 0; kb < NKB; ++kb)
#pragma unroll
        for (int j = 0; j < 8; ++j)
#pragma unroll
            for (int c = 0; c < 4; ++c) {
                if (VL && kb >= nkv) break;
                const int r = c >> 1;
                float e = fast_ex2(s[kb][4 * j + c] - mx[r]);
                l[r] += e;
                if (!((keep[kb][r] >> (8 * j + (c & 1))) & 1ull)) e = 0.f;
                s[kb][4 * j + c] = e;
            }
#pragma unroll
    for (int r = 0; r < 2; ++r) {
        l[r] += __shfl_xor_sync(0xffffffffu, l[r], 1);
        l[r] += __shfl_xor_sync(0xffffffffu, l[r], 2);
    }

    uint32_t pa[NKB][4][4];
#pragma unroll
    for (int kb = 0; kb < NKB; ++kb)
#pragma unroll
        for (int kk = 0; kk < 4; ++kk)
            if (!VL || kb < nkv) pack_afrag(pa[kb][kk], s[kb], kk);
    float o[32];
    wgmma_fence();
#pragma unroll
    for (int kb = 0; kb < NKB; ++kb)
#pragma unroll
        for (int kk = 0; kk < 4; ++kk)
            if (!VL || kb < nkv)
                wgmma_m64n64k16_rs<1>(o, pa[kb][kk], tile_desc(sV + kb * kWgTile + kk * 2048), (kb > 0 || kk > 0) ? 1u : 0u);
    wgmma_commit();
    wgmma_wait<0>();

    const float dscale = p.drop_scale != 0.f ? p.drop_scale : 1.f;
    store_rows(p.ctx + (VL ? sp.row0 : static_cast<long long>(b) * S) * p.H + h * kHd, p.H, q0, S, o, t, dscale / l[0], dscale / l[1]);
    if (t == 0 && p.lse != nullptr) {
        float* lse = p.lse + (VL ? sp.stat0 : static_cast<long long>(item) * S);
        if (q0 < S) lse[q0] = (mx[0] + log2f(l[0])) * 0.6931471805599453f;
        if (q0 + 8 < S) lse[q0 + 8] = (mx[1] + log2f(l[1])) * 0.6931471805599453f;
    }
}

template <int NKB, bool VL = false>
__global__ void __launch_bounds__(NKB * 128, 1)
attn_bwd_wgmma_kernel(const __grid_constant__ CUtensorMap tmQKV, const __grid_constant__ CUtensorMap tmDO, const AttnParams p) {
    extern __shared__ uint8_t smem_raw[];
    const uint32_t raw = smem_u32(smem_raw);
    const uint32_t base = (raw + 1023u) & ~1023u;
    uint8_t* smem = smem_raw + (base - raw);
    const uint32_t sQ = base, sK = base + NKB * kWgTile, sV = base + 2 * NKB * kWgTile, sDO = base + 3 * NKB * kWgTile;
    const uint32_t sPS = base + 4 * NKB * kWgTile;
    float* sbias = reinterpret_cast<float*>(smem + (4 * NKB + NKB * NKB) * kWgTile);
    const uint32_t bar = base + (4 * NKB + NKB * NKB) * kWgTile + NKB * kBlk * 4;
    const int tid = threadIdx.x, wg = tid >> 7, warp = (tid >> 5) & 3, lane = tid & 31, g = lane >> 2, t = lane & 3;
    const int item = blockIdx.x, b = item / p.A, h = item % p.A;
    const unsigned bh = static_cast<unsigned>(item);
    const long long ld = 3LL * p.H;
    const SeqSpan sp = seq_span<VL>(p, b, h);
    const int S = sp.len;
    const int nkv = VL ? (S + kBlk - 1) / kBlk : NKB;
    const int row0 = VL ? static_cast<int>(sp.row0) : b * S;
    const long long stat0 = VL ? sp.stat0 : static_cast<long long>(item) * S;
    if (VL && S == 0) return;
    const bool wg_live = !VL || wg < nkv;

    if (tid == 0) {
        tma_prefetch_desc(&tmQKV);
        tma_prefetch_desc(&tmDO);
        mbar_init(bar, 1);
        fence_barrier_init();
    }
    __syncthreads();
    pdl_trigger();
    pdl_wait();
    if (tid == 0) {
        mbar_arrive_expect_tx(bar, 4 * nkv * kWgTile);
#pragma unroll
        for (int kb = 0; kb < NKB; ++kb) {
            if (VL && kb >= nkv) break;
#pragma unroll
            for (int m = 0; m < 3; ++m) tma_load_2d(base + (m * NKB + kb) * kWgTile, &tmQKV, bar, m * p.H + h * kHd, row0 + kb * kBlk);
            tma_load_2d(sDO + kb * kWgTile, &tmDO, bar, h * kHd, row0 + kb * kBlk);
        }
    }
    for (int i = tid; i < NKB * kBlk; i += NKB * 128) sbias[i] = key_bias2<VL>(p, b, i, S);
    const int r0 = warp * 16 + g;
    const int q0 = wg * kBlk + r0;
    float lse2[2], dr[2];
#pragma unroll
    for (int r = 0; r < 2; ++r) {
        const int q = q0 + 8 * r;
        lse2[r] = q < S ? p.lse[stat0 + q] * kLog2e : INFINITY;
        dr[r] = q < S ? p.drow[stat0 + q] : 0.f;
    }
    unsigned long long keep[NKB][2];
#pragma unroll
    for (int kb = 0; kb < NKB; ++kb) {
        keep[kb][0] = keep_word(p, bh, q0, kb, NKB, t);
        keep[kb][1] = keep_word(p, bh, q0 + 8, kb, NKB, t);
    }
    __syncthreads();
    mbar_wait(bar, 0);
    const float sc2 = p.scale * kLog2e;
    const float ds = p.drop_scale != 0.f ? p.drop_scale : 1.f;
    auto probs = [&](float (&s)[32], int kb) {
#pragma unroll
        for (int j = 0; j < 8; ++j)
#pragma unroll
            for (int c = 0; c < 4; ++c)
                s[4 * j + c] = fast_ex2(fmaf(s[4 * j + c], sc2, sbias[kb * kBlk + 8 * j + 2 * t + (c & 1)]) - lse2[c >> 1]);
    };
    auto kept = [&](int kb, int j, int c) { return ((keep[kb][c >> 1] >> (8 * j + (c & 1))) & 1ull) != 0; };
    bf16* dqkv = p.dqkv + (VL ? sp.row0 : static_cast<long long>(b) * S) * ld + h * kHd;

#pragma unroll
    for (int kb = 0; kb < NKB; ++kb) {
        if (VL && (!wg_live || kb >= nkv)) break;
        float s[32];
        wgmma_fence();
        qk_block<NKB>(s, sQ, sK, wg, kb);
        wgmma_commit();
        wgmma_wait<0>();
        probs(s, kb);
#pragma unroll
        for (int j = 0; j < 8; ++j)
#pragma unroll
            for (int c = 0; c < 4; ++c) s[4 * j + c] = kept(kb, j, c) ? s[4 * j + c] * ds : 0.f;
        store_tile(sPS + (wg * NKB + kb) * kWgTile, r0, s, t);
    }
    fence_proxy_async_smem();
    __syncthreads();
    if (wg_live) {
        float acc[32];
        wgmma_fence();
#pragma unroll
        for (int qb = 0; qb < NKB; ++qb)
#pragma unroll
            for (int kk = 0; kk < 4; ++kk)
                if (!VL || qb < nkv)
                    wgmma_m64n64k16_ss<1, 1>(acc, tile_desc(sPS + (qb * NKB + wg) * kWgTile + kk * 2048),
                                             tile_desc(sDO + qb * kWgTile + kk * 2048), (qb > 0 || kk > 0) ? 1u : 0u);
        wgmma_commit();
        wgmma_wait<0>();
        store_rows(dqkv + 2 * p.H, ld, q0, S, acc, t, 1.f, 1.f);
    }
    __syncthreads();

    float dq[32];
#pragma unroll
    for (int kb = 0; kb < NKB; ++kb) {
        if (VL && (!wg_live || kb >= nkv)) break;
        float s[32], dp[32];
        wgmma_fence();
        qk_block<NKB>(s, sQ, sK, wg, kb);
#pragma unroll
        for (int k = 0; k < kHd / 16; ++k)
            wgmma_m64n64k16_ss<0, 0>(dp, tile_desc(sDO + wg * kWgTile + k * 32), tile_desc(sV + kb * kWgTile + k * 32), k > 0 ? 1u : 0u);
        wgmma_commit();
        wgmma_wait<0>();
        probs(s, kb);
#pragma unroll
        for (int j = 0; j < 8; ++j)
#pragma unroll
            for (int c = 0; c < 4; ++c) {
                const float dpd = kept(kb, j, c) ? dp[4 * j + c] * ds : 0.f;
                s[4 * j + c] *= dpd - dr[c >> 1];
            }
        store_tile(sPS + (wg * NKB + kb) * kWgTile, r0, s, t);
        uint32_t pa[4][4];
#pragma unroll
        for (int kk = 0; kk < 4; ++kk) pack_afrag(pa[kk], s, kk);
        wgmma_fence();
#pragma unroll
        for (int kk = 0; kk < 4; ++kk)
            wgmma_m64n64k16_rs<1>(dq, pa[kk], tile_desc(sK + kb * kWgTile + kk * 2048), (kb > 0 || kk > 0) ? 1u : 0u);
        wgmma_commit();
        wgmma_wait<0>();
    }
    if (wg_live) store_rows(dqkv, ld, q0, S, dq, t, p.scale, p.scale);
    fence_proxy_async_smem();
    __syncthreads();
    if (wg_live) {
        float acc[32];
        wgmma_fence();
#pragma unroll
        for (int qb = 0; qb < NKB; ++qb)
#pragma unroll
            for (int kk = 0; kk < 4; ++kk)
                if (!VL || qb < nkv)
                    wgmma_m64n64k16_ss<1, 1>(acc, tile_desc(sPS + (qb * NKB + wg) * kWgTile + kk * 2048),
                                             tile_desc(sQ + qb * kWgTile + kk * 2048), (qb > 0 || kk > 0) ? 1u : 0u);
        wgmma_commit();
        wgmma_wait<0>();
        store_rows(dqkv + p.H, ld, q0, S, acc, t, p.scale, p.scale);
    }
}

template <int NKB, bool VL = false>
static int launch_fwd_wgmma(const AttnParams& p, const CUtensorMap& tq, cudaStream_t st) {
    auto kern = attn_fwd_wgmma_kernel<NKB, VL>;
    static int configured[kMaxDevices] = {0};
    VB_CHECK_CUDA(ensure_dyn_smem(kern, AttnSmem<NKB>::FWD_BYTES, configured));
    ProfScope ps(st, PROF_ATTN_FWD, 4.0 * p.B * p.A * p.S * p.S * kHd, 1);
    VB_CHECK_CUDA(launch_pdl(kern, dim3(p.B * p.A), dim3(NKB * 128), AttnSmem<NKB>::FWD_BYTES, st, tq, p));
    return 0;
}
template <int NKB, bool VL = false>
static int launch_bwd_wgmma(const AttnParams& p, const CUtensorMap& tq, const CUtensorMap& td, cudaStream_t st) {
    auto kern = attn_bwd_wgmma_kernel<NKB, VL>;
    static int configured[kMaxDevices] = {0};
    VB_CHECK_CUDA(ensure_dyn_smem(kern, AttnSmem<NKB>::BWD_BYTES, configured));
    ProfScope ps(st, PROF_ATTN_DKV, 10.0 * p.B * p.A * p.S * p.S * kHd, 1);
    VB_CHECK_CUDA(launch_pdl(kern, dim3(p.B * p.A), dim3(NKB * 128), AttnSmem<NKB>::BWD_BYTES, st, tq, td, p));
    return 0;
}

int attn_fwd_wgmma(const AttnParams& p, const AttnDropOffset& off, cudaStream_t st) {
    const int nkb = (p.S + kBlk - 1) / kBlk;
    int rc = attn_keep_mask(p, off, nkb, st);
    if (rc) return rc;
    CUtensorMap tq;
    const bool vl = p.cu_seqlens != nullptr;
    const uint64_t rows = vl ? static_cast<uint64_t>(p.total) : static_cast<uint64_t>(p.B) * p.S;
    rc = make_tmap_bf16(&tq, p.qkv, 3ull * p.H, rows, 3ull * p.H, kBlk);
    if (rc) return rc;
    if (vl) {
        if (nkb == 1) rc = launch_fwd_wgmma<1, true>(p, tq, st);
        else if (nkb == 2) rc = launch_fwd_wgmma<2, true>(p, tq, st);
        else rc = launch_fwd_wgmma<3, true>(p, tq, st);
    } else if (nkb == 1) rc = launch_fwd_wgmma<1>(p, tq, st);
    else if (nkb == 2) rc = launch_fwd_wgmma<2>(p, tq, st);
    else rc = launch_fwd_wgmma<3>(p, tq, st);
    if (rc) return rc;
    VB_CHECK_CUDA(cudaGetLastError());
    return 0;
}

int attn_bwd_wgmma(const AttnParams& p, cudaStream_t st, bool delta_ready) {
    const int nkb = (p.S + kBlk - 1) / kBlk;
    int rc = 0;
    if (!delta_ready) {
        rc = attn_delta(p, st);
        if (rc) return rc;
    }
    CUtensorMap tq, td;
    const bool vl = p.cu_seqlens != nullptr;
    const uint64_t rows = vl ? static_cast<uint64_t>(p.total) : static_cast<uint64_t>(p.B) * p.S;
    rc = make_tmap_bf16(&tq, p.qkv, 3ull * p.H, rows, 3ull * p.H, kBlk);
    if (rc) return rc;
    rc = make_tmap_bf16(&td, p.dctx, static_cast<uint64_t>(p.H), rows, static_cast<uint64_t>(p.H), kBlk);
    if (rc) return rc;
    if (vl) {
        if (nkb == 1) rc = launch_bwd_wgmma<1, true>(p, tq, td, st);
        else if (nkb == 2) rc = launch_bwd_wgmma<2, true>(p, tq, td, st);
        else rc = launch_bwd_wgmma<3, true>(p, tq, td, st);
    } else if (nkb == 1) rc = launch_bwd_wgmma<1>(p, tq, td, st);
    else if (nkb == 2) rc = launch_bwd_wgmma<2>(p, tq, td, st);
    else rc = launch_bwd_wgmma<3>(p, tq, td, st);
    if (rc) return rc;
    VB_CHECK_CUDA(cudaGetLastError());
    return 0;
}

}
```

### visualbert_b200/csrc/vb_common.cuh

```cuda
#pragma once

#include <cuda.h>
#include <cuda_bf16.h>
#include <cuda_runtime.h>
#include <stdint.h>
#include <stdio.h>

#include <atomic>

namespace vb {

typedef __nv_bfloat16 bf16;

extern std::atomic<long long> g_launches;
int num_sms();
constexpr int kMaxDevices = 64;
int current_device();
struct DetWs { void* ptr; long long bytes; };
DetWs det_ws();
int det_require(long long need, const char* what);
const unsigned long long* drop_offset();
template <typename K>
inline cudaError_t ensure_dyn_smem(K kern, int bytes, int (&cache)[kMaxDevices]) {
    const int d = current_device();
    if (cache[d] >= bytes) return cudaSuccess;
    cudaError_t e = cudaFuncSetAttribute(kern, cudaFuncAttributeMaxDynamicSharedMemorySize, bytes);
    if (e == cudaSuccess) cache[d] = bytes;
    return e;
}

enum { PROF_GEMM_FWD = 0, PROF_GEMM_DGRAD = 1, PROF_GEMM_WGRAD = 2, PROF_ATTN_FWD = 3, PROF_ATTN_DQ = 4, PROF_ATTN_DKV = 5,
       PROF_LN_FWD = 6, PROF_LN_BWD = 7, PROF_COLSUM = 8, PROF_EMBED = 9, PROF_OTHER = 10, PROF_NCAT = 11 };
#ifdef __CUDACC__
__device__ __forceinline__ void pdl_wait() { asm volatile("griddepcontrol.wait;" ::: "memory"); }
__device__ __forceinline__ void pdl_trigger() { asm volatile("griddepcontrol.launch_dependents;" ::: "memory"); }
template <typename... KArgs, typename... Args>
inline cudaError_t launch_pdl(void (*kernel)(KArgs...), dim3 grid, dim3 block, size_t smem, cudaStream_t st, Args&&... args) {
    cudaLaunchConfig_t cfg = {};
    cfg.gridDim = grid;
    cfg.blockDim = block;
    cfg.dynamicSmemBytes = smem;
    cfg.stream = st;
    cudaLaunchAttribute attr[1];
    attr[0].id = cudaLaunchAttributeProgrammaticStreamSerialization;
    attr[0].val.programmaticStreamSerializationAllowed = 1;
    cfg.attrs = attr;
    cfg.numAttrs = 1;
    return cudaLaunchKernelEx(&cfg, kernel, static_cast<KArgs>(args)...);
}
#endif

struct ProfScope {
    ProfScope(cudaStream_t st, int cat, double work, int launches);
    ~ProfScope();
    int slot;
    cudaStream_t st;
};

void set_error(const char* fmt, ...);
#define VB_CHECK_CUDA(expr)                                                                   \
    do {                                                                                      \
        cudaError_t _e = (expr);                                                              \
        if (_e != cudaSuccess) {                                                              \
            vb::set_error("%s:%d: %s -> %s", __FILE__, __LINE__, #expr, cudaGetErrorString(_e)); \
            return 1;                                                                         \
        }                                                                                     \
    } while (0)
#define VB_REQUIRE(cond, ...)                                                                 \
    do {                                                                                      \
        if (!(cond)) {                                                                        \
            vb::set_error(__VA_ARGS__);                                                       \
            return 2;                                                                         \
        }                                                                                     \
    } while (0)

#define VB_TRY_RC(expr)      \
    do {                     \
        int _rc = (expr);    \
        if (_rc) return _rc; \
    } while (0)

template <typename... T>
inline bool all_aligned16(const T*... p) {
    return ((reinterpret_cast<uintptr_t>(p) | ... | uintptr_t{0}) & 15) == 0;
}

__device__ __forceinline__ uint32_t smem_u32(const void* p) {
    return static_cast<uint32_t>(__cvta_generic_to_shared(p));
}

__device__ __forceinline__ float warp_sum(float v) {
#pragma unroll
    for (int o = 16; o > 0; o >>= 1) v += __shfl_xor_sync(0xffffffffu, v, o);
    return v;
}
__device__ __forceinline__ float warp_max(float v) {
#pragma unroll
    for (int o = 16; o > 0; o >>= 1) v = fmaxf(v, __shfl_xor_sync(0xffffffffu, v, o));
    return v;
}

__device__ __forceinline__ uint32_t pack_bf16x2(float lo, float hi) {
    __nv_bfloat162 h = __floats2bfloat162_rn(lo, hi);
    return *reinterpret_cast<uint32_t*>(&h);
}
__device__ __forceinline__ float2 unpack_bf16x2(uint32_t v) {
    __nv_bfloat162 h = *reinterpret_cast<__nv_bfloat162*>(&v);
    return __bfloat1622float2(h);
}

__device__ __forceinline__ float fast_ex2(float x) {
    float r;
    asm("ex2.approx.ftz.f32 %0, %1;" : "=f"(r) : "f"(x));
    return r;
}
__device__ __forceinline__ float fast_rcp(float x) {
    float r;
    asm("rcp.approx.ftz.f32 %0, %1;" : "=f"(r) : "f"(x));
    return r;
}

__device__ __forceinline__ float erfc_abs_sqrt2(float x, float& e) {
    const float ax = fabsf(x);
    e = fast_ex2(x * x * -0.72134752044448170f);
    const float t = fast_rcp(fmaf(0.23164189f, ax, 1.0f));
    float poly = fmaf(1.061405429f, t, -1.453152027f);
    poly = fmaf(poly, t, 1.421413741f);
    poly = fmaf(poly, t, -0.284496736f);
    poly = fmaf(poly, t, 0.254829592f);
    return poly * t * e;
}
__device__ __forceinline__ float gelu_fwd(float x) {
    float e;
    const float q = erfc_abs_sqrt2(x, e);
    const float hx = 0.5f * x, ha = fabsf(hx);
    return fmaf(-ha, q, hx + ha);
}
__device__ __forceinline__ void gelu_fwd_bwd(float x, float& g, float& gp) {
    float e;
    const float q = erfc_abs_sqrt2(x, e);
    const float cdf = 0.5f + copysignf(fmaf(-0.5f, q, 0.5f), x);
    g = x * cdf;
    gp = fmaf(x * e, 0.3989422804014327f, cdf);
}
__device__ __forceinline__ float gelu_bwd(float x) {
    float e;
    const float q = erfc_abs_sqrt2(x, e);
    const float cdf = 0.5f + copysignf(fmaf(-0.5f, q, 0.5f), x);
    return fmaf(x * e, 0.3989422804014327f, cdf);
}

__device__ __forceinline__ uint32_t mix32(uint32_t x) {
    x ^= x >> 16; x *= 0x7feb352du;
    x ^= x >> 15; x *= 0x846ca68bu;
    x ^= x >> 16;
    return x;
}
__device__ __forceinline__ uint32_t dropout_key(uint64_t seed, uint32_t stream) {
    return mix32(static_cast<uint32_t>(seed) ^ mix32(static_cast<uint32_t>(seed >> 32) + 0x9E3779B9u * (stream + 1u)));
}
struct DropQ { unsigned thr8; float scale; };
inline DropQ dropout_quantise(float p) {
    DropQ q;
    unsigned n = static_cast<unsigned>(p * 256.0f + 0.5f);
    if (n > 255u) n = 255u;
    q.thr8 = n;
    q.scale = p > 0.f ? 256.0f / (256.0f - static_cast<float>(n)) : 0.f;
    return q;
}
__device__ __forceinline__ uint32_t dropout_keep8_key(uint32_t key0, uint64_t elem8, uint32_t thr8) {
    const uint32_t key = key0 ^ (static_cast<uint32_t>(elem8 >> 31) * 0x27d4eb2fu);
    const uint32_t base = static_cast<uint32_t>(elem8) << 1;
    const uint32_t t4 = thr8 * 0x01010101u;
    const uint32_t m0 = __vcmpgeu4(mix32(base ^ key), t4) & 0x01010101u;
    const uint32_t m1 = __vcmpgeu4(mix32((base + 1u) ^ key), t4) & 0x01010101u;
    return ((m0 * 0x01020408u) >> 24) | (((m1 * 0x01020408u) >> 24) << 4);
}
__device__ __forceinline__ uint32_t dropout_keep8(uint64_t seed, uint32_t stream, uint64_t elem8, uint32_t thr8) {
    return dropout_keep8_key(dropout_key(seed, stream), elem8, thr8);
}

__device__ __forceinline__ void mbar_init(uint32_t bar, uint32_t count) {
    asm volatile("mbarrier.init.shared::cta.b64 [%0], %1;" ::"r"(bar), "r"(count) : "memory");
}
__device__ __forceinline__ void fence_barrier_init() {
    asm volatile("fence.mbarrier_init.release.cluster;" ::: "memory");
}
__device__ __forceinline__ void fence_proxy_async_smem() {
    asm volatile("fence.proxy.async.shared::cta;" ::: "memory");
}
__device__ __forceinline__ void mbar_arrive(uint32_t bar) {
    asm volatile("mbarrier.arrive.shared::cta.b64 _, [%0];" ::"r"(bar) : "memory");
}
__device__ __forceinline__ void mbar_arrive_expect_tx(uint32_t bar, uint32_t bytes) {
    asm volatile("mbarrier.arrive.expect_tx.shared::cta.b64 _, [%0], %1;" ::"r"(bar), "r"(bytes)
                 : "memory");
}
__device__ __forceinline__ bool mbar_try_wait(uint32_t bar, uint32_t parity) {
    uint32_t ok;
    asm volatile(
        "{\n"
        ".reg .pred p;\n"
        "mbarrier.try_wait.parity.shared::cta.b64 p, [%1], %2;\n"
        "selp.u32 %0, 1, 0, p;\n"
        "}\n"
        : "=r"(ok)
        : "r"(bar), "r"(parity)
        : "memory");
    return ok != 0;
}
__device__ __forceinline__ void mbar_wait(uint32_t bar, uint32_t parity) {
    if (mbar_try_wait(bar, parity)) return;
    const long long t0 = clock64();
    uint32_t spins = 0;
    while (!mbar_try_wait(bar, parity)) {
        if ((++spins & 0x3ffu) == 0 && clock64() - t0 > 4000000000ll) __trap();
    }
}

__device__ __forceinline__ void tma_prefetch_desc(const CUtensorMap* m) {
    asm volatile("prefetch.tensormap [%0];" ::"l"(reinterpret_cast<uint64_t>(m)) : "memory");
}
__device__ __forceinline__ void tma_load_2d(uint32_t smem_dst, const CUtensorMap* m, uint32_t bar,
                                            int c_inner, int c_outer) {
    asm volatile(
        "cp.async.bulk.tensor.2d.shared::cluster.global.mbarrier::complete_tx::bytes"
        " [%0], [%1, {%3, %4}], [%2];"
        ::"r"(smem_dst), "l"(reinterpret_cast<uint64_t>(m)), "r"(bar), "r"(c_inner), "r"(c_outer)
        : "memory");
}

__device__ __forceinline__ uint64_t wgmma_desc_sw128(uint32_t saddr, uint32_t lbo_bytes, uint32_t sbo_bytes) {
    return static_cast<uint64_t>((saddr & 0x3FFFFu) >> 4) | (static_cast<uint64_t>((lbo_bytes >> 4) & 0x3FFFu) << 16) |
           (static_cast<uint64_t>((sbo_bytes >> 4) & 0x3FFFu) << 32) | (1ull << 62);
}
__device__ __forceinline__ void wgmma_fence() { asm volatile("wgmma.fence.sync.aligned;" ::: "memory"); }
__device__ __forceinline__ void wgmma_commit() { asm volatile("wgmma.commit_group.sync.aligned;" ::: "memory"); }
template <int N>
__device__ __forceinline__ void wgmma_wait() { asm volatile("wgmma.wait_group.sync.aligned %0;" ::"n"(N) : "memory"); }
template <int TA, int TB>
__device__ __forceinline__ void wgmma_m64n128k16(float (&d)[64], uint64_t a_desc, uint64_t b_desc, uint32_t accumulate) {
    asm volatile(
        "{\n"
        ".reg .pred p;\n"
        "setp.ne.b32 p, %66, 0;\n"
        "wgmma.mma_async.sync.aligned.m64n128k16.f32.bf16.bf16 "
        "{%0, %1, %2, %3, %4, %5, %6, %7, %8, %9, %10, %11, %12, %13, %14, %15, %16, %17, %18, %19, %20, %21, %22, %23, %24, %25, %26, %27, %28, %29, %30, %31, %32, %33, %34, %35, %36, %37, %38, %39, %40, %41, %42, %43, %44, %45, %46, %47, %48, %49, %50, %51, %52, %53, %54, %55, %56, %57, %58, %59, %60, %61, %62, %63}, "
        "%64, %65, p, 1, 1, %67, %68;\n"
        "}\n"
        : "+f"(d[0]), "+f"(d[1]), "+f"(d[2]), "+f"(d[3]), "+f"(d[4]), "+f"(d[5]), "+f"(d[6]), "+f"(d[7]),
          "+f"(d[8]), "+f"(d[9]), "+f"(d[10]), "+f"(d[11]), "+f"(d[12]), "+f"(d[13]), "+f"(d[14]), "+f"(d[15]),
          "+f"(d[16]), "+f"(d[17]), "+f"(d[18]), "+f"(d[19]), "+f"(d[20]), "+f"(d[21]), "+f"(d[22]), "+f"(d[23]),
          "+f"(d[24]), "+f"(d[25]), "+f"(d[26]), "+f"(d[27]), "+f"(d[28]), "+f"(d[29]), "+f"(d[30]), "+f"(d[31]),
          "+f"(d[32]), "+f"(d[33]), "+f"(d[34]), "+f"(d[35]), "+f"(d[36]), "+f"(d[37]), "+f"(d[38]), "+f"(d[39]),
          "+f"(d[40]), "+f"(d[41]), "+f"(d[42]), "+f"(d[43]), "+f"(d[44]), "+f"(d[45]), "+f"(d[46]), "+f"(d[47]),
          "+f"(d[48]), "+f"(d[49]), "+f"(d[50]), "+f"(d[51]), "+f"(d[52]), "+f"(d[53]), "+f"(d[54]), "+f"(d[55]),
          "+f"(d[56]), "+f"(d[57]), "+f"(d[58]), "+f"(d[59]), "+f"(d[60]), "+f"(d[61]), "+f"(d[62]), "+f"(d[63])
        : "l"(a_desc), "l"(b_desc), "r"(accumulate), "n"(TA), "n"(TB));
}
template <int TA, int TB>
__device__ __forceinline__ void wgmma_m64n64k16_ss(float (&d)[32], uint64_t a_desc, uint64_t b_desc, uint32_t accumulate) {
    asm volatile(
        "{\n"
        ".reg .pred p;\n"
        "setp.ne.b32 p, %34, 0;\n"
        "wgmma.mma_async.sync.aligned.m64n64k16.f32.bf16.bf16 "
        "{%0, %1, %2, %3, %4, %5, %6, %7, %8, %9, %10, %11, %12, %13, %14, %15, %16, %17, %18, %19, %20, %21, %22, %23, %24, %25, %26, %27, %28, %29, %30, %31}, "
        "%32, %33, p, 1, 1, %35, %36;\n"
        "}\n"
        : "+f"(d[0]), "+f"(d[1]), "+f"(d[2]), "+f"(d[3]), "+f"(d[4]), "+f"(d[5]), "+f"(d[6]), "+f"(d[7]),
          "+f"(d[8]), "+f"(d[9]), "+f"(d[10]), "+f"(d[11]), "+f"(d[12]), "+f"(d[13]), "+f"(d[14]), "+f"(d[15]),
          "+f"(d[16]), "+f"(d[17]), "+f"(d[18]), "+f"(d[19]), "+f"(d[20]), "+f"(d[21]), "+f"(d[22]), "+f"(d[23]),
          "+f"(d[24]), "+f"(d[25]), "+f"(d[26]), "+f"(d[27]), "+f"(d[28]), "+f"(d[29]), "+f"(d[30]), "+f"(d[31])
        : "l"(a_desc), "l"(b_desc), "r"(accumulate), "n"(TA), "n"(TB));
}
template <int TB>
__device__ __forceinline__ void wgmma_m64n64k16_rs(float (&d)[32], const uint32_t (&a)[4], uint64_t b_desc, uint32_t accumulate) {
    asm volatile(
        "{\n"
        ".reg .pred p;\n"
        "setp.ne.b32 p, %37, 0;\n"
        "wgmma.mma_async.sync.aligned.m64n64k16.f32.bf16.bf16 "
        "{%0, %1, %2, %3, %4, %5, %6, %7, %8, %9, %10, %11, %12, %13, %14, %15, %16, %17, %18, %19, %20, %21, %22, %23, %24, %25, %26, %27, %28, %29, %30, %31}, "
        "{%32, %33, %34, %35}, %36, p, 1, 1, %38;\n"
        "}\n"
        : "+f"(d[0]), "+f"(d[1]), "+f"(d[2]), "+f"(d[3]), "+f"(d[4]), "+f"(d[5]), "+f"(d[6]), "+f"(d[7]),
          "+f"(d[8]), "+f"(d[9]), "+f"(d[10]), "+f"(d[11]), "+f"(d[12]), "+f"(d[13]), "+f"(d[14]), "+f"(d[15]),
          "+f"(d[16]), "+f"(d[17]), "+f"(d[18]), "+f"(d[19]), "+f"(d[20]), "+f"(d[21]), "+f"(d[22]), "+f"(d[23]),
          "+f"(d[24]), "+f"(d[25]), "+f"(d[26]), "+f"(d[27]), "+f"(d[28]), "+f"(d[29]), "+f"(d[30]), "+f"(d[31])
        : "r"(a[0]), "r"(a[1]), "r"(a[2]), "r"(a[3]), "l"(b_desc), "r"(accumulate), "n"(TB));
}
__device__ __forceinline__ bool elect_one() {
    uint32_t pred;
    asm volatile(
        "{\n"
        ".reg .pred P1;\n"
        "elect.sync _|P1, 0xffffffff;\n"
        "selp.u32 %0, 1, 0, P1;\n"
        "}\n"
        : "=r"(pred));
    return pred != 0;
}
template <int N>
__device__ __forceinline__ void reg_dec() { asm volatile("setmaxnreg.dec.sync.aligned.u32 %0;" ::"n"(N)); }
template <int N>
__device__ __forceinline__ void reg_inc() { asm volatile("setmaxnreg.inc.sync.aligned.u32 %0;" ::"n"(N)); }
__device__ __forceinline__ void named_bar_sync(int id, int nthreads) {
    asm volatile("bar.sync %0, %1;" ::"r"(id), "r"(nthreads) : "memory");
}

__device__ __forceinline__ uint4 ldg_v4(const void* p) {
    return __ldg(reinterpret_cast<const uint4*>(p));
}
__device__ __forceinline__ void stg_v4(void* p, uint4 v) { *reinterpret_cast<uint4*>(p) = v; }
__device__ __forceinline__ void ldg_v8(const void* p, uint32_t (&r)[8]) {
    const uint4 a = ldg_v4(p), b = ldg_v4(static_cast<const uint8_t*>(p) + 16);
    r[0] = a.x; r[1] = a.y; r[2] = a.z; r[3] = a.w; r[4] = b.x; r[5] = b.y; r[6] = b.z; r[7] = b.w;
}
__device__ __forceinline__ void stg_v8(void* p, const uint32_t (&r)[8]) {
    stg_v4(p, make_uint4(r[0], r[1], r[2], r[3]));
    stg_v4(static_cast<uint8_t*>(p) + 16, make_uint4(r[4], r[5], r[6], r[7]));
}
__device__ __forceinline__ void red_add_v4_f32(float* p, float a, float b, float c, float d) {
    asm volatile("red.global.add.v4.f32 [%0], {%1, %2, %3, %4};" ::"l"(p), "f"(a), "f"(b), "f"(c),
                 "f"(d)
                 : "memory");
}

}
```

### visualbert_b200/csrc/vb_internal.h

```cpp
#pragma once
#include "../../include/vbert_b200.h"
#include "vb_common.cuh"

namespace vb {

int gemm(const vb_gemm_args& a, cudaStream_t st);
bool gemm_gp_tiled_ok(int M, int N);
bool gemm_delta_ok(int M, int N);
int ln_fwd(const void* x, long long ldx, const float* gamma, const float* beta, void* y, long long ldy, float* mean,
           float* rstd, int rows, int H, float eps, cudaStream_t st);
int ln_bwd(const void* dy, const void* x, const float* mean, const float* rstd, const float* gamma, void* dx,
           void* dx_drop, float* dgamma, float* dbeta, float* dbias, int rows, int H, float dropout_p,
           unsigned long long seed, unsigned stream_id, float in_dropout_p, unsigned in_stream_id, cudaStream_t st);
enum class AttnRoute { Wgmma, Head, Staged };
inline AttnRoute attn_route(int S) { return S <= 192 ? AttnRoute::Wgmma : S <= 256 ? AttnRoute::Head : AttnRoute::Staged; }
int attn_fwd(const void* qkv, const float* mask_bias, void* ctx, float* lse, void* keep, int B, int S, int A, int H,
             float dropout_p, unsigned long long seed, unsigned stream_id, cudaStream_t st);
int attn_bwd(const void* qkv, const float* mask_bias, const void* ctx, const float* lse, const void* keep,
             const void* dctx, void* dqkv, float* drow, int B, int S, int A, int H, float dropout_p,
             unsigned long long seed, unsigned stream_id, cudaStream_t st, bool delta_ready = false);
int attn_fwd_varlen(const void* qkv, const int* cu_seqlens, void* ctx, float* lse, void* keep, int B, int max_seq, int total,
                    int A, int H, float dropout_p, unsigned long long seed, unsigned stream_id, cudaStream_t st, bool need_lse = true);
int attn_bwd_varlen(const void* qkv, const int* cu_seqlens, const void* ctx, const float* lse, const void* keep,
                    const void* dctx, void* dqkv, float* drow, int B, int max_seq, int total, int A, int H, float dropout_p,
                    unsigned long long seed, unsigned stream_id, cudaStream_t st, bool delta_ready = false);
long long attn_keep_bytes(int B, int S, int A);
int attn_probs(const void* qkv, const float* mask_bias, float* probs, int B, int S, int A, int H, cudaStream_t st);
int wgrad_splits(long long tiles, int k_blocks);
long long gemm_tiles(int M, int N);
int gemm_k_blocks(int K);
long long ln_bwd_det_bytes(int rows, int H);
long long colsum_det_bytes(int M, int N);
long long embed_bwd_det_bytes(int B, int T, int V, int H, long long sort_temp);
long long embed_sort_temp_bytes(int B, int T, int V);
int partials_reduce(const float* part, int parts, int width, int seg, float* o0, float* o1, float* o2, cudaStream_t st);
int colsum(const void* x, long long ld, float* out, int M, int N, cudaStream_t st);
int cast_f32_bf16(const float* src, void* dst, long long n, cudaStream_t st);
int cast_bf16_f32(const void* src, float* dst, long long n, cudaStream_t st);
int mask_bias(const long long* input_mask, const long long* image_mask, float* out, int B, int T, int V, cudaStream_t st);

struct EmbedParams {
    const long long* ids; const long long* tt; const long long* vt;
    const bf16* vis_proj;
    const float* word; const float* pos; const float* type; const float* pos_vis; const float* type_vis;
    const float* gamma; const float* beta;
    bf16* pre; bf16* y; float* mean; float* rstd;
    int B, T, V, H, vocab, max_pos, n_types;
    float eps;
    float drop_scale; unsigned drop_thresh16; unsigned long long drop_seed; unsigned drop_stream;
    const unsigned long long* drop_offset;
};
struct EmbedBwdParams {
    const bf16* de;
    const long long* ids; const long long* tt; const long long* vt;
    float* dword; float* dpos; float* dtype; float* dpos_vis; float* dtype_vis;
    bf16* dvis;
    int B, T, V, H, vocab, max_pos, n_types;
};
int embed_fwd(const EmbedParams& p, cudaStream_t st);
int embed_bwd(const EmbedBwdParams& p, cudaStream_t st);


}
```

Measured before the change: 4301.

## Make wgmma attention kernels persistent with double-buffered loads and fused QKV bias grad

Forward and backward wgmma attention kernels become persistent, with the grid capped at the SM count. Each block loops over (batch, head) items and prefetches the next item's Q/K/V tiles, keep-mask (via bulk async copy) and key bias into a second buffer while computing the current one. The backward kernel also accumulates the QKV bias gradient via per-warp column sums in shared memory, which removes the separate colsum pass over dQKV when deterministic workspace is off. This costs more shared memory and makes the bias gradient depend on how its atomic/flush accumulation is ordered.

```diff
diff --git a/visualbert_b200/csrc/vb_api.cu b/visualbert_b200/csrc/vb_api.cu
--- a/visualbert_b200/csrc/vb_api.cu
+++ b/visualbert_b200/csrc/vb_api.cu
@@ -126,14 +126,16 @@
     const bool fused_delta = gemm_delta_ok(M, H) && w->drow != nullptr && attn_route(d->seq) != AttnRoute::Staged;
     if (fused_delta) { a.delta_ctx = s->ctx; a.delta_out = w->drow; a.delta_seq = vl ? rows.total : d->seq; }
     VB_TRY(gemm(a, st));
+    const bool fused_dbias = attn_route(d->seq) == AttnRoute::Wgmma && det_ws().ptr == nullptr;
+    float* db_qkv = fused_dbias ? g->db_qkv : nullptr;
     if (vl)
         VB_TRY(attn_bwd_varlen(s->qkv, rows.cu_seqlens, s->ctx, s->lse, s->keep_mask, w->d_ctx, w->d_big, w->drow, d->batch, d->seq,
                                rows.total, d->heads, H, d->attn_dropout, d->seed, drop_stream(d->layer_index, kSiteAttnProbs), st,
-                               fused_delta));
+                               fused_delta, db_qkv));
     else
         VB_TRY(attn_bwd(s->qkv, d->mask_bias, s->ctx, s->lse, s->keep_mask, w->d_ctx, w->d_big, w->drow, d->batch, d->seq, d->heads, H,
-                        d->attn_dropout, d->seed, drop_stream(d->layer_index, kSiteAttnProbs), st, fused_delta));
-    VB_TRY(colsum(w->d_big, 3 * H, g->db_qkv, M, 3 * H, st));
+                        d->attn_dropout, d->seed, drop_stream(d->layer_index, kSiteAttnProbs), st, fused_delta, db_qkv));
+    if (!fused_dbias) VB_TRY(colsum(w->d_big, 3 * H, g->db_qkv, M, 3 * H, st));
     VB_TRY(gemm(wgrad_args(w->d_big, x_in, g->dw_qkv, M, 3 * H, H), st));
     a = dgrad_args(w->d_big, d->w_qkv, dx, M, 3 * H, H);
     a.addend = w->d_pre; a.ld_add = H;
diff --git a/visualbert_b200/csrc/vb_attention.cu b/visualbert_b200/csrc/vb_attention.cu
--- a/visualbert_b200/csrc/vb_attention.cu
+++ b/visualbert_b200/csrc/vb_attention.cu
@@ -428,6 +428,7 @@
     p.B = B; p.S = S; p.A = A; p.H = H;
     p.cu_seqlens = nullptr;
     p.total = 0;
+    p.dbias = nullptr;
     p.scale = 0.125f;
     const unsigned th8 = static_cast<unsigned>(dropout_p * 256.f + 0.5f);
     p.drop_thresh16 = th8;
@@ -510,6 +511,7 @@
     const int B = p.B, S = p.S, A = p.A;
     dim3 grid((S + kBlk - 1) / kBlk, A, B);
     const AttnRoute route = attn_route(S);
+    VB_REQUIRE(p.dbias == nullptr || route == AttnRoute::Wgmma, "attention backward: dbias is only computed for seq <= 192");
     if (route == AttnRoute::Wgmma) return attn_bwd_wgmma(p, st, delta_ready);
     if (route == AttnRoute::Head) return attn_bwd_head(p, static_cast<int>(grid.x), st, delta_ready);
     const int nsub = static_cast<int>(grid.x) < kMaxSub ? static_cast<int>(grid.x) : kMaxSub;
@@ -538,21 +540,23 @@
 
 int attn_bwd(const void* qkv, const float* mask_bias, const void* ctx, const float* lse, const void* keep,
              const void* dctx, void* dqkv, float* drow, int B, int S, int A, int H, float dropout_p,
-             unsigned long long seed, unsigned stream_id, cudaStream_t st, bool delta_ready) {
+             unsigned long long seed, unsigned stream_id, cudaStream_t st, bool delta_ready, float* dbias) {
     AttnParams p;
     int rc = fill_params(p, qkv, mask_bias, const_cast<void*>(ctx), const_cast<float*>(lse), dctx, dqkv, drow,
                          const_cast<void*>(keep), B, S, A, H, dropout_p, seed, stream_id);
     if (rc) return rc;
+    p.dbias = dbias;
     return attn_bwd_launch(p, st, delta_ready);
 }
 
 int attn_bwd_varlen(const void* qkv, const int* cu_seqlens, const void* ctx, const float* lse, const void* keep,
                     const void* dctx, void* dqkv, float* drow, int B, int max_seq, int total, int A, int H, float dropout_p,
-                    unsigned long long seed, unsigned stream_id, cudaStream_t st, bool delta_ready) {
+                    unsigned long long seed, unsigned stream_id, cudaStream_t st, bool delta_ready, float* dbias) {
     AttnParams p;
     int rc = fill_params(p, qkv, nullptr, const_cast<void*>(ctx), const_cast<float*>(lse), dctx, dqkv, drow,
                          const_cast<void*>(keep), B, max_seq, A, H, dropout_p, seed, stream_id);
     if (rc) return rc;
+    p.dbias = dbias;
     VB_REQUIRE(ctx && lse && dctx && drow, "attention varlen: null pointer");
     if ((rc = set_varlen(p, cu_seqlens, total, qkv, dqkv))) return rc;
     if (total == 0) return 0;
diff --git a/visualbert_b200/csrc/vb_attention.cuh b/visualbert_b200/csrc/vb_attention.cuh
--- a/visualbert_b200/csrc/vb_attention.cuh
+++ b/visualbert_b200/csrc/vb_attention.cuh
@@ -27,6 +27,7 @@
     unsigned drop_seed;
     const int* cu_seqlens;
     int total;
+    float* dbias;
 };
 
 struct SeqSpan {
diff --git a/visualbert_b200/csrc/vb_attention_wgmma.cu b/visualbert_b200/csrc/vb_attention_wgmma.cu
--- a/visualbert_b200/csrc/vb_attention_wgmma.cu
+++ b/visualbert_b200/csrc/vb_attention_wgmma.cu
@@ -6,16 +6,19 @@
 
 template <int NKB>
 struct AttnSmem {
-    static constexpr int FWD_BYTES = 3 * NKB * kWgTile + NKB * kBlk * 4 + 16 + 1024;
-    static constexpr int BWD_BYTES = (4 * NKB + NKB * NKB) * kWgTile + NKB * kBlk * 4 + 16 + 1024;
+    static constexpr int KEEP = NKB * kBlk * NKB * 8;
+    static constexpr int BIAS = NKB * kBlk * 4;
+    static constexpr int F_TILES = 3 * NKB * kWgTile;
+    static constexpr int F_KEEP = 2 * F_TILES, F_BIAS = F_KEEP + 2 * KEEP, F_BAR = F_BIAS + 2 * BIAS;
+    static constexpr int FWD_BYTES = F_BAR + 16 + 1024;
+    static constexpr int B_QK = 2 * NKB * kWgTile;
+    static constexpr int B_V = 2 * B_QK, B_DO = B_V + NKB * kWgTile, B_PS = B_DO + NKB * kWgTile;
+    static constexpr int B_BIAS = B_PS + NKB * NKB * kWgTile, B_KEEP = B_BIAS + 2 * BIAS, B_DB = B_KEEP + KEEP;
+    static constexpr int B_BAR = B_DB + NKB * 4 * kHd * 4;
+    static constexpr int BWD_BYTES = B_BAR + 24 + 1024;
 };
 
 __device__ __forceinline__ uint64_t tile_desc(uint32_t saddr) { return wgmma_desc_sw128(saddr, kWgTile, 1024); }
-
-__device__ __forceinline__ unsigned long long keep_word(const AttnParams& p, unsigned bh, int q, int kb, int nkb, int t) {
-    if (p.drop_scale == 0.f) return ~0ull;
-    return p.keep[(static_cast<unsigned long long>(bh) * (nkb * kBlk) + q) * nkb + kb] >> (2 * t);
-}
 
 template <int NKB>
 __device__ __forceinline__ void qk_block(float (&s)[32], uint32_t sQ, uint32_t sK, int wg, int kb) {
@@ -38,6 +41,20 @@
             *reinterpret_cast<uint32_t*>(base + static_cast<long long>(r0 + 8) * ld + col) = pack_bf16x2(x[4 * j + 2] * mul1, x[4 * j + 3] * mul1);
     }
 }
+__device__ __forceinline__ void colsum_rows(float* sums, int r0, int nrows, const float (&x)[32], int g, int t, float mul) {
+#pragma unroll
+    for (int j = 0; j < 8; ++j)
+#pragma unroll
+        for (int c = 0; c < 2; ++c) {
+            const float a = r0 < nrows ? __bfloat162float(__float2bfloat16_rn(x[4 * j + c] * mul)) : 0.f;
+            const float b = r0 + 8 < nrows ? __bfloat162float(__float2bfloat16_rn(x[4 * j + 2 + c] * mul)) : 0.f;
+            float v = a + b;
+            v += __shfl_xor_sync(0xffffffffu, v, 4);
+            v += __shfl_xor_sync(0xffffffffu, v, 8);
+            v += __shfl_xor_sync(0xffffffffu, v, 16);
+            if (g == 0) sums[8 * j + 2 * t + c] = v;
+        }
+}
 __device__ __forceinline__ void store_tile(uint32_t tile, int r, const float (&x)[32], int t) {
 #pragma unroll
     for (int j = 0; j < 8; ++j) {
@@ -45,60 +62,42 @@
         st_shared_u32(tile + swz(r + 8, j) + 4 * t, pack_bf16x2(x[4 * j + 2], x[4 * j + 3]));
     }
 }
-
-template <int NKB, bool VL = false>
-__global__ void __launch_bounds__(NKB * 128, 1)
-attn_fwd_wgmma_kernel(const __grid_constant__ CUtensorMap tmQKV, const AttnParams p) {
-    extern __shared__ uint8_t smem_raw[];
-    const uint32_t raw = smem_u32(smem_raw);
-    const uint32_t base = (raw + 1023u) & ~1023u;
-    uint8_t* smem = smem_raw + (base - raw);
-    const uint32_t sQ = base, sK = base + NKB * kWgTile, sV = base + 2 * NKB * kWgTile;
-    float* sbias = reinterpret_cast<float*>(smem + 3 * NKB * kWgTile);
-    const uint32_t bar = base + 3 * NKB * kWgTile + NKB * kBlk * 4;
-    const int tid = threadIdx.x, wg = tid >> 7, warp = (tid >> 5) & 3, lane = tid & 31, g = lane >> 2, t = lane & 3;
-    const int item = blockIdx.x, b = item / p.A, h = item % p.A;
-    const unsigned bh = static_cast<unsigned>(item);
-    const SeqSpan sp = seq_span<VL>(p, b, h);
-    const int S = sp.len;
-    const int nkv = VL ? (S + kBlk - 1) / kBlk : NKB;
-    const int row0 = VL ? static_cast<int>(sp.row0) : b * S;
-    if (VL && S == 0) return;
-
-    if (tid == 0) {
-        tma_prefetch_desc(&tmQKV);
-        mbar_init(bar, 1);
-        fence_barrier_init();
-    }
-    __syncthreads();
-    pdl_trigger();
-    pdl_wait();
-    if (tid == 0) {
-        mbar_arrive_expect_tx(bar, 3 * nkv * kWgTile);
-#pragma unroll
-        for (int m = 0; m < 3; ++m)
-#pragma unroll
-            for (int kb = 0; kb < NKB; ++kb)
-                if (!VL || kb < nkv) tma_load_2d(base + (m * NKB + kb) * kWgTile, &tmQKV, bar, m * p.H + h * kHd, row0 + kb * kBlk);
-    }
-    for (int i = tid; i < NKB * kBlk; i += NKB * 128) sbias[i] = key_bias2<VL>(p, b, i, S);
-    const int q0 = wg * kBlk + warp * 16 + g;
-    unsigned long long keep[NKB][2];
-#pragma unroll
-    for (int kb = 0; kb < NKB; ++kb) {
-        keep[kb][0] = keep_word(p, bh, q0, kb, NKB, t);
-        keep[kb][1] = keep_word(p, bh, q0 + 8, kb, NKB, t);
-    }
-    __syncthreads();
+template <int NKB, bool VL>
+__device__ __forceinline__ int live_blocks(int len) { return VL ? (len + kBlk - 1) / kBlk : NKB; }
+
+template <int NKB, bool VL>
+__device__ __forceinline__ void fwd_issue(const CUtensorMap* tm, const AttnParams& p, int item, const SeqSpan& sp, uint32_t tiles,
+                                          uint32_t keep, uint32_t bar) {
+    const int h = item % p.A, nkv = live_blocks<NKB, VL>(sp.len);
+    const bool drop = p.drop_scale != 0.f && nkv > 0;
+    mbar_arrive_expect_tx(bar, 3 * nkv * kWgTile + (drop ? AttnSmem<NKB>::KEEP : 0));
+#pragma unroll
+    for (int m = 0; m < 3; ++m)
+#pragma unroll
+        for (int kb = 0; kb < NKB; ++kb)
+            if (kb < nkv) tma_load_2d(tiles + (m * NKB + kb) * kWgTile, tm, bar, m * p.H + (h * kHd), static_cast<int>(sp.row0) + kb * kBlk);
+    if (drop) bulk_load(keep, p.keep + static_cast<unsigned long long>(item) * (NKB * kBlk * NKB), AttnSmem<NKB>::KEEP, bar);
+}
+
+template <int NKB, bool VL>
+__device__ __forceinline__ void fwd_head(const AttnParams& p, uint32_t sQ, const unsigned long long* skeep, const float* sbias, int h,
+                                         const SeqSpan& sp, int wg, int q0, int t) {
+    const int S = sp.len, nkv = live_blocks<NKB, VL>(S);
     if (VL && wg >= nkv) return;
-    mbar_wait(bar, 0);
-
+    const uint32_t sK = sQ + NKB * kWgTile, sV = sQ + 2 * NKB * kWgTile;
     float s[NKB][32];
     wgmma_fence();
 #pragma unroll
     for (int kb = 0; kb < NKB; ++kb)
         if (!VL || kb < nkv) qk_block<NKB>(s[kb], sQ, sK, wg, kb);
     wgmma_commit();
+    const bool drop = p.drop_scale != 0.f;
+    unsigned long long keep[NKB][2];
+#pragma unroll
+    for (int kb = 0; kb < NKB; ++kb) {
+        keep[kb][0] = drop ? skeep[q0 * NKB + kb] >> (2 * t) : ~0ull;
+        keep[kb][1] = drop ? skeep[(q0 + 8) * NKB + kb] >> (2 * t) : ~0ull;
+    }
     wgmma_wait<0>();
 
     const float sc2 = p.scale * kLog2e;
@@ -156,10 +155,10 @@
     wgmma_commit();
     wgmma_wait<0>();
 
-    const float dscale = p.drop_scale != 0.f ? p.drop_scale : 1.f;
-    store_rows(p.ctx + (VL ? sp.row0 : static_cast<long long>(b) * S) * p.H + h * kHd, p.H, q0, S, o, t, dscale / l[0], dscale / l[1]);
+    const float dscale = drop ? p.drop_scale : 1.f;
+    store_rows(p.ctx + sp.row0 * p.H + h * kHd, p.H, q0, S, o, t, dscale / l[0], dscale / l[1]);
     if (t == 0 && p.lse != nullptr) {
-        float* lse = p.lse + (VL ? sp.stat0 : static_cast<long long>(item) * S);
+        float* lse = p.lse + sp.stat0;
         if (q0 < S) lse[q0] = (mx[0] + log2f(l[0])) * 0.6931471805599453f;
         if (q0 + 8 < S) lse[q0 + 8] = (mx[1] + log2f(l[1])) * 0.6931471805599453f;
     }
@@ -167,156 +166,275 @@
 
 template <int NKB, bool VL = false>
 __global__ void __launch_bounds__(NKB * 128, 1)
-attn_bwd_wgmma_kernel(const __grid_constant__ CUtensorMap tmQKV, const __grid_constant__ CUtensorMap tmDO, const AttnParams p) {
+attn_fwd_wgmma_kernel(const __grid_constant__ CUtensorMap tmQKV, const AttnParams p) {
+    using SM = AttnSmem<NKB>;
     extern __shared__ uint8_t smem_raw[];
     const uint32_t raw = smem_u32(smem_raw);
     const uint32_t base = (raw + 1023u) & ~1023u;
     uint8_t* smem = smem_raw + (base - raw);
-    const uint32_t sQ = base, sK = base + NKB * kWgTile, sV = base + 2 * NKB * kWgTile, sDO = base + 3 * NKB * kWgTile;
-    const uint32_t sPS = base + 4 * NKB * kWgTile;
-    float* sbias = reinterpret_cast<float*>(smem + (4 * NKB + NKB * NKB) * kWgTile);
-    const uint32_t bar = base + (4 * NKB + NKB * NKB) * kWgTile + NKB * kBlk * 4;
+    auto skeep = [&](int buf) { return reinterpret_cast<const unsigned long long*>(smem + SM::F_KEEP + buf * SM::KEEP); };
+    auto sbias = [&](int buf) { return reinterpret_cast<float*>(smem + SM::F_BIAS + buf * SM::BIAS); };
+    auto bar = [&](int buf) { return base + SM::F_BAR + 8 * buf; };
     const int tid = threadIdx.x, wg = tid >> 7, warp = (tid >> 5) & 3, lane = tid & 31, g = lane >> 2, t = lane & 3;
-    const int item = blockIdx.x, b = item / p.A, h = item % p.A;
-    const unsigned bh = static_cast<unsigned>(item);
+    const int q0 = wg * kBlk + warp * 16 + g;
+    const int items = p.B * p.A;
+
+    if (tid == 0) {
+        tma_prefetch_desc(&tmQKV);
+        mbar_init(bar(0), 1);
+        mbar_init(bar(1), 1);
+        fence_barrier_init();
+    }
+    __syncthreads();
+    pdl_trigger();
+    pdl_wait();
+    {
+        const int item = blockIdx.x;
+        const SeqSpan sp = seq_span<VL>(p, item / p.A, item % p.A);
+        if (tid == 0) fwd_issue<NKB, VL>(&tmQKV, p, item, sp, base, base + SM::F_KEEP, bar(0));
+        if (tid < NKB * kBlk) sbias(0)[tid] = key_bias2<VL>(p, item / p.A, tid, sp.len);
+    }
+    for (int i = 0, item = blockIdx.x; item < items; ++i, item += gridDim.x) {
+        const int buf = i & 1, next = item + gridDim.x;
+        const bool more = next < items;
+        float bias_next = 0.f;
+        __syncthreads();
+        if (more && (tid == 0 || tid < NKB * kBlk)) {
+            const SeqSpan spn = seq_span<VL>(p, next / p.A, next % p.A);
+            if (tid == 0) fwd_issue<NKB, VL>(&tmQKV, p, next, spn, base + (buf ^ 1) * SM::F_TILES, base + SM::F_KEEP + (buf ^ 1) * SM::KEEP,
+                                             bar(buf ^ 1));
+            if (tid < NKB * kBlk) bias_next = key_bias2<VL>(p, next / p.A, tid, spn.len);
+        }
+        mbar_wait(bar(buf), (i >> 1) & 1);
+        fwd_head<NKB, VL>(p, base + buf * SM::F_TILES, skeep(buf), sbias(buf), item % p.A, seq_span<VL>(p, item / p.A, item % p.A), wg, q0, t);
+        if (more && tid < NKB * kBlk) sbias(buf ^ 1)[tid] = bias_next;
+    }
+}
+
+template <int NKB, bool VL = false>
+__global__ void __launch_bounds__(NKB * 128, 1)
+attn_bwd_wgmma_kernel(const __grid_constant__ CUtensorMap tmQKV, const __grid_constant__ CUtensorMap tmDO, const AttnParams p) {
+    using SM = AttnSmem<NKB>;
+    extern __shared__ uint8_t smem_raw[];
+    const uint32_t raw = smem_u32(smem_raw);
+    const uint32_t base = (raw + 1023u) & ~1023u;
+    uint8_t* smem = smem_raw + (base - raw);
+    const uint32_t sV = base + SM::B_V, sDO = base + SM::B_DO;
+    const uint32_t sPS = base + SM::B_PS;
+    auto sbias = [&](int buf) { return reinterpret_cast<float*>(smem + SM::B_BIAS + buf * SM::BIAS); };
+    const unsigned long long* skeep = reinterpret_cast<const unsigned long long*>(smem + SM::B_KEEP);
+    float* sdb = reinterpret_cast<float*>(smem + SM::B_DB);
+    auto bar_qk = [&](int buf) { return base + SM::B_BAR + 8 * buf; };
+    const uint32_t bar_vd = base + SM::B_BAR + 16;
+    const int tid = threadIdx.x, wg = tid >> 7, warp = (tid >> 5) & 3, lane = tid & 31, g = lane >> 2, t = lane & 3;
+    const int r0 = warp * 16 + g;
+    const int q0 = wg * kBlk + r0;
     const long long ld = 3LL * p.H;
-    const SeqSpan sp = seq_span<VL>(p, b, h);
-    const int S = sp.len;
-    const int nkv = VL ? (S + kBlk - 1) / kBlk : NKB;
-    const int row0 = VL ? static_cast<int>(sp.row0) : b * S;
-    const long long stat0 = VL ? sp.stat0 : static_cast<long long>(item) * S;
-    if (VL && S == 0) return;
-    const bool wg_live = !VL || wg < nkv;
+    const int items = p.B * p.A;
+    const float sc2 = p.scale * kLog2e;
+    const bool drop = p.drop_scale != 0.f;
+    const float ds = drop ? p.drop_scale : 1.f;
 
     if (tid == 0) {
         tma_prefetch_desc(&tmQKV);
         tma_prefetch_desc(&tmDO);
-        mbar_init(bar, 1);
+        mbar_init(bar_qk(0), 1);
+        mbar_init(bar_qk(1), 1);
+        mbar_init(bar_vd, 1);
         fence_barrier_init();
     }
     __syncthreads();
     pdl_trigger();
     pdl_wait();
+
+    auto issue_qk = [&](int item, const SeqSpan& sp, int buf) {
+        const int h = item % p.A, nkv = live_blocks<NKB, VL>(sp.len);
+        mbar_arrive_expect_tx(bar_qk(buf), 2 * nkv * kWgTile);
+#pragma unroll
+        for (int m = 0; m < 2; ++m)
+#pragma unroll
+            for (int kb = 0; kb < NKB; ++kb)
+                if (kb < nkv)
+                    tma_load_2d(base + buf * SM::B_QK + (m * NKB + kb) * kWgTile, &tmQKV, bar_qk(buf), m * p.H + h * kHd,
+                                static_cast<int>(sp.row0) + kb * kBlk);
+    };
+    auto issue_vd = [&](int item, const SeqSpan& sp) {
+        const int h = item % p.A, nkv = live_blocks<NKB, VL>(sp.len);
+        const bool kw = drop && nkv > 0;
+        mbar_arrive_expect_tx(bar_vd, 2 * nkv * kWgTile + (kw ? SM::KEEP : 0));
+#pragma unroll
+        for (int kb = 0; kb < NKB; ++kb)
+            if (kb < nkv) {
+                tma_load_2d(sV + kb * kWgTile, &tmQKV, bar_vd, 2 * p.H + h * kHd, static_cast<int>(sp.row0) + kb * kBlk);
+                tma_load_2d(sDO + kb * kWgTile, &tmDO, bar_vd, h * kHd, static_cast<int>(sp.row0) + kb * kBlk);
+            }
+        if (kw) bulk_load(base + SM::B_KEEP, p.keep + static_cast<unsigned long long>(item) * (NKB * kBlk * NKB), SM::KEEP, bar_vd);
+    };
+    float lse2[2], dr[2];
+    auto load_rows = [&](int item, const SeqSpan& sp) {
+#pragma unroll
+        for (int r = 0; r < 2; ++r) {
+            const int q = q0 + 8 * r;
+            lse2[r] = q < sp.len ? p.lse[sp.stat0 + q] * kLog2e : INFINITY;
+            dr[r] = q < sp.len ? p.drow[sp.stat0 + q] : 0.f;
+        }
+    };
+    auto flush_dbias = [&](int m, int h, int nkv) {
+        if (tid < kHd) {
+            float v = 0.f;
+            for (int w = 0; w < 4 * nkv; ++w) v += sdb[w * kHd + tid];
+            atomicAdd(p.dbias + m * p.H + h * kHd + tid, v);
+        }
+    };
+
+    int item = blockIdx.x;
+    SeqSpan sp = seq_span<VL>(p, item / p.A, item % p.A);
     if (tid == 0) {
-        mbar_arrive_expect_tx(bar, 4 * nkv * kWgTile);
-#pragma unroll
-        for (int kb = 0; kb < NKB; ++kb) {
-            if (VL && kb >= nkv) break;
-#pragma unroll
-            for (int m = 0; m < 3; ++m) tma_load_2d(base + (m * NKB + kb) * kWgTile, &tmQKV, bar, m * p.H + h * kHd, row0 + kb * kBlk);
-            tma_load_2d(sDO + kb * kWgTile, &tmDO, bar, h * kHd, row0 + kb * kBlk);
-        }
-    }
-    for (int i = tid; i < NKB * kBlk; i += NKB * 128) sbias[i] = key_bias2<VL>(p, b, i, S);
-    const int r0 = warp * 16 + g;
-    const int q0 = wg * kBlk + r0;
-    float lse2[2], dr[2];
-#pragma unroll
-    for (int r = 0; r < 2; ++r) {
-        const int q = q0 + 8 * r;
-        lse2[r] = q < S ? p.lse[stat0 + q] * kLog2e : INFINITY;
-        dr[r] = q < S ? p.drow[stat0 + q] : 0.f;
-    }
-    unsigned long long keep[NKB][2];
-#pragma unroll
-    for (int kb = 0; kb < NKB; ++kb) {
-        keep[kb][0] = keep_word(p, bh, q0, kb, NKB, t);
-        keep[kb][1] = keep_word(p, bh, q0 + 8, kb, NKB, t);
-    }
-    __syncthreads();
-    mbar_wait(bar, 0);
-    const float sc2 = p.scale * kLog2e;
-    const float ds = p.drop_scale != 0.f ? p.drop_scale : 1.f;
-    auto probs = [&](float (&s)[32], int kb) {
-#pragma unroll
-        for (int j = 0; j < 8; ++j)
-#pragma unroll
-            for (int c = 0; c < 4; ++c)
-                s[4 * j + c] = fast_ex2(fmaf(s[4 * j + c], sc2, sbias[kb * kBlk + 8 * j + 2 * t + (c & 1)]) - lse2[c >> 1]);
-    };
-    auto kept = [&](int kb, int j, int c) { return ((keep[kb][c >> 1] >> (8 * j + (c & 1))) & 1ull) != 0; };
-    bf16* dqkv = p.dqkv + (VL ? sp.row0 : static_cast<long long>(b) * S) * ld + h * kHd;
-
-#pragma unroll
-    for (int kb = 0; kb < NKB; ++kb) {
-        if (VL && (!wg_live || kb >= nkv)) break;
-        float s[32];
-        wgmma_fence();
-        qk_block<NKB>(s, sQ, sK, wg, kb);
-        wgmma_commit();
-        wgmma_wait<0>();
-        probs(s, kb);
-#pragma unroll
-        for (int j = 0; j < 8; ++j)
-#pragma unroll
-            for (int c = 0; c < 4; ++c) s[4 * j + c] = kept(kb, j, c) ? s[4 * j + c] * ds : 0.f;
-        store_tile(sPS + (wg * NKB + kb) * kWgTile, r0, s, t);
-    }
-    fence_proxy_async_smem();
-    __syncthreads();
-    if (wg_live) {
-        float acc[32];
-        wgmma_fence();
-#pragma unroll
-        for (int qb = 0; qb < NKB; ++qb)
-#pragma unroll
-            for (int kk = 0; kk < 4; ++kk)
-                if (!VL || qb < nkv)
-                    wgmma_m64n64k16_ss<1, 1>(acc, tile_desc(sPS + (qb * NKB + wg) * kWgTile + kk * 2048),
-                                             tile_desc(sDO + qb * kWgTile + kk * 2048), (qb > 0 || kk > 0) ? 1u : 0u);
-        wgmma_commit();
-        wgmma_wait<0>();
-        store_rows(dqkv + 2 * p.H, ld, q0, S, acc, t, 1.f, 1.f);
-    }
-    __syncthreads();
-
-    float dq[32];
-#pragma unroll
-    for (int kb = 0; kb < NKB; ++kb) {
-        if (VL && (!wg_live || kb >= nkv)) break;
-        float s[32], dp[32];
-        wgmma_fence();
-        qk_block<NKB>(s, sQ, sK, wg, kb);
-#pragma unroll
-        for (int k = 0; k < kHd / 16; ++k)
-            wgmma_m64n64k16_ss<0, 0>(dp, tile_desc(sDO + wg * kWgTile + k * 32), tile_desc(sV + kb * kWgTile + k * 32), k > 0 ? 1u : 0u);
-        wgmma_commit();
-        wgmma_wait<0>();
-        probs(s, kb);
-#pragma unroll
-        for (int j = 0; j < 8; ++j)
-#pragma unroll
-            for (int c = 0; c < 4; ++c) {
-                const float dpd = kept(kb, j, c) ? dp[4 * j + c] * ds : 0.f;
-                s[4 * j + c] *= dpd - dr[c >> 1];
+        issue_qk(item, sp, 0);
+        issue_vd(item, sp);
+    }
+    if (tid < NKB * kBlk) sbias(0)[tid] = key_bias2<VL>(p, item / p.A, tid, sp.len);
+    load_rows(item, sp);
+    int h_flush = -1, nkv_flush = 0;
+    for (int i = 0; item < items; ++i, item += gridDim.x) {
+        const int buf = i & 1, next = item + gridDim.x, h = item % p.A;
+        const bool more = next < items;
+        const SeqSpan spn = more ? seq_span<VL>(p, next / p.A, next % p.A) : sp;
+        const int S = sp.len, nkv = live_blocks<NKB, VL>(S);
+        const bool wg_live = !VL || wg < nkv;
+        const uint32_t sQ = base + buf * SM::B_QK, sK = sQ + NKB * kWgTile;
+        const float* sb = sbias(buf);
+        bf16* dqkv = p.dqkv + sp.row0 * ld + h * kHd;
+        __syncthreads();
+        if (tid == 0 && more) issue_qk(next, spn, buf ^ 1);
+        if (h_flush >= 0) flush_dbias(1, h_flush, nkv_flush);
+        const bool db = p.dbias != nullptr && S > 0;
+        h_flush = db ? h : -1;
+        nkv_flush = nkv;
+        mbar_wait(bar_qk(buf), (i >> 1) & 1);
+        mbar_wait(bar_vd, i & 1);
+        auto probs = [&](float (&s)[32], int kb) {
+#pragma unroll
+            for (int j = 0; j < 8; ++j)
+#pragma unroll
+                for (int c = 0; c < 4; ++c)
+                    s[4 * j + c] = fast_ex2(fmaf(s[4 * j + c], sc2, sb[kb * kBlk + 8 * j + 2 * t + (c & 1)]) - lse2[c >> 1]);
+        };
+        auto keep_words = [&](unsigned long long (&w)[2], int kb) {
+            w[0] = drop ? skeep[q0 * NKB + kb] >> (2 * t) : ~0ull;
+            w[1] = drop ? skeep[(q0 + 8) * NKB + kb] >> (2 * t) : ~0ull;
+        };
+        auto kept = [&](const unsigned long long (&w)[2], int j, int c) { return ((w[c >> 1] >> (8 * j + (c & 1))) & 1ull) != 0; };
+
+        float dq[32], acc[32];
+        if (S > 0) {
+#pragma unroll
+            for (int kb = 0; kb < NKB; ++kb) {
+                if (VL && (!wg_live || kb >= nkv)) break;
+                float s[32];
+                wgmma_fence();
+                qk_block<NKB>(s, sQ, sK, wg, kb);
+                wgmma_commit();
+                unsigned long long kw[2];
+                keep_words(kw, kb);
+                wgmma_wait<0>();
+                probs(s, kb);
+#pragma unroll
+                for (int j = 0; j < 8; ++j)
+#pragma unroll
+                    for (int c = 0; c < 4; ++c) s[4 * j + c] = kept(kw, j, c) ? s[4 * j + c] * ds : 0.f;
+                store_tile(sPS + (wg * NKB + kb) * kWgTile, r0, s, t);
             }
-        store_tile(sPS + (wg * NKB + kb) * kWgTile, r0, s, t);
-        uint32_t pa[4][4];
-#pragma unroll
-        for (int kk = 0; kk < 4; ++kk) pack_afrag(pa[kk], s, kk);
-        wgmma_fence();
-#pragma unroll
-        for (int kk = 0; kk < 4; ++kk)
-            wgmma_m64n64k16_rs<1>(dq, pa[kk], tile_desc(sK + kb * kWgTile + kk * 2048), (kb > 0 || kk > 0) ? 1u : 0u);
-        wgmma_commit();
-        wgmma_wait<0>();
-    }
-    if (wg_live) store_rows(dqkv, ld, q0, S, dq, t, p.scale, p.scale);
-    fence_proxy_async_smem();
-    __syncthreads();
-    if (wg_live) {
-        float acc[32];
-        wgmma_fence();
-#pragma unroll
-        for (int qb = 0; qb < NKB; ++qb)
-#pragma unroll
-            for (int kk = 0; kk < 4; ++kk)
-                if (!VL || qb < nkv)
-                    wgmma_m64n64k16_ss<1, 1>(acc, tile_desc(sPS + (qb * NKB + wg) * kWgTile + kk * 2048),
-                                             tile_desc(sQ + qb * kWgTile + kk * 2048), (qb > 0 || kk > 0) ? 1u : 0u);
-        wgmma_commit();
-        wgmma_wait<0>();
-        store_rows(dqkv + p.H, ld, q0, S, acc, t, p.scale, p.scale);
+            fence_proxy_async_smem();
+            __syncthreads();
+            if (wg_live) {
+                wgmma_fence();
+#pragma unroll
+                for (int qb = 0; qb < NKB; ++qb)
+#pragma unroll
+                    for (int kk = 0; kk < 4; ++kk)
+                        if (!VL || qb < nkv)
+                            wgmma_m64n64k16_ss<1, 1>(acc, tile_desc(sPS + (qb * NKB + wg) * kWgTile + kk * 2048),
+                                                     tile_desc(sDO + qb * kWgTile + kk * 2048), (qb > 0 || kk > 0) ? 1u : 0u);
+                wgmma_commit();
+                wgmma_wait<0>();
+                store_rows(dqkv + 2 * p.H, ld, q0, S, acc, t, 1.f, 1.f);
+                if (db) colsum_rows(sdb + (tid >> 5) * kHd, q0, S, acc, g, t, 1.f);
+            }
+            __syncthreads();
+            if (db) flush_dbias(2, h, nkv);
+
+#pragma unroll
+            for (int kb = 0; kb < NKB; ++kb) {
+                if (VL && (!wg_live || kb >= nkv)) break;
+                float s[32], dp[32];
+                wgmma_fence();
+                qk_block<NKB>(s, sQ, sK, wg, kb);
+#pragma unroll
+                for (int k = 0; k < kHd / 16; ++k)
+                    wgmma_m64n64k16_ss<0, 0>(dp, tile_desc(sDO + wg * kWgTile + k * 32), tile_desc(sV + kb * kWgTile + k * 32), k > 0 ? 1u : 0u);
+                wgmma_commit();
+                unsigned long long kw[2];
+                keep_words(kw, kb);
+                wgmma_wait<0>();
+                probs(s, kb);
+#pragma unroll
+                for (int j = 0; j < 8; ++j)
+#pragma unroll
+                    for (int c = 0; c < 4; ++c) {
+                        const float dpd = kept(kw, j, c) ? dp[4 * j + c] * ds : 0.f;
+                        s[4 * j + c] *= dpd - dr[c >> 1];
+                    }
+                store_tile(sPS + (wg * NKB + kb) * kWgTile, r0, s, t);
+                uint32_t pa[4][4];
+#pragma unroll
+                for (int kk = 0; kk < 4; ++kk) pack_afrag(pa[kk], s, kk);
+                wgmma_fence();
+#pragma unroll
+                for (int kk = 0; kk < 4; ++kk)
+                    wgmma_m64n64k16_rs<1>(dq, pa[kk], tile_desc(sK + kb * kWgTile + kk * 2048), (kb > 0 || kk > 0) ? 1u : 0u);
+                wgmma_commit();
+                wgmma_wait<0>();
+            }
+            if (wg_live) store_rows(dqkv, ld, q0, S, dq, t, p.scale, p.scale);
+            fence_proxy_async_smem();
+        }
+        __syncthreads();
+        if (db) {
+            if (wg_live) colsum_rows(sdb + (tid >> 5) * kHd, q0, S, dq, g, t, p.scale);
+            __syncthreads();
+            flush_dbias(0, h, nkv);
+        }
+        float bias_next = 0.f;
+        if (more) {
+            if (tid == 0) issue_vd(next, spn);
+            if (tid < NKB * kBlk) bias_next = key_bias2<VL>(p, next / p.A, tid, spn.len);
+            load_rows(next, spn);
+        }
+
+        if (S > 0 && wg_live) {
+            wgmma_fence();
+#pragma unroll
+            for (int qb = 0; qb < NKB; ++qb)
+#pragma unroll
+                for (int kk = 0; kk < 4; ++kk)
+                    if (!VL || qb < nkv)
+                        wgmma_m64n64k16_ss<1, 1>(acc, tile_desc(sPS + (qb * NKB + wg) * kWgTile + kk * 2048),
+                                                 tile_desc(sQ + qb * kWgTile + kk * 2048), (qb > 0 || kk > 0) ? 1u : 0u);
+            wgmma_commit();
+            wgmma_wait<0>();
+            store_rows(dqkv + p.H, ld, q0, S, acc, t, p.scale, p.scale);
+        }
+        if (db) {
+            __syncthreads();
+            if (wg_live) colsum_rows(sdb + (tid >> 5) * kHd, q0, S, acc, g, t, p.scale);
+        }
+        if (more && tid < NKB * kBlk) sbias(buf ^ 1)[tid] = bias_next;
+        sp = spn;
+    }
+    if (h_flush >= 0) {
+        __syncthreads();
+        flush_dbias(1, h_flush, nkv_flush);
     }
 }
 
@@ -325,8 +443,9 @@
     auto kern = attn_fwd_wgmma_kernel<NKB, VL>;
     static int configured[kMaxDevices] = {0};
     VB_CHECK_CUDA(ensure_dyn_smem(kern, AttnSmem<NKB>::FWD_BYTES, configured));
+    const int items = p.B * p.A, grid = items < num_sms() ? items : num_sms();
     ProfScope ps(st, PROF_ATTN_FWD, 4.0 * p.B * p.A * p.S * p.S * kHd, 1);
-    VB_CHECK_CUDA(launch_pdl(kern, dim3(p.B * p.A), dim3(NKB * 128), AttnSmem<NKB>::FWD_BYTES, st, tq, p));
+    VB_CHECK_CUDA(launch_pdl(kern, dim3(grid), dim3(NKB * 128), AttnSmem<NKB>::FWD_BYTES, st, tq, p));
     return 0;
 }
 template <int NKB, bool VL = false>
@@ -334,13 +453,15 @@
     auto kern = attn_bwd_wgmma_kernel<NKB, VL>;
     static int configured[kMaxDevices] = {0};
     VB_CHECK_CUDA(ensure_dyn_smem(kern, AttnSmem<NKB>::BWD_BYTES, configured));
+    const int items = p.B * p.A, grid = items < num_sms() ? items : num_sms();
     ProfScope ps(st, PROF_ATTN_DKV, 10.0 * p.B * p.A * p.S * p.S * kHd, 1);
-    VB_CHECK_CUDA(launch_pdl(kern, dim3(p.B * p.A), dim3(NKB * 128), AttnSmem<NKB>::BWD_BYTES, st, tq, td, p));
+    VB_CHECK_CUDA(launch_pdl(kern, dim3(grid), dim3(NKB * 128), AttnSmem<NKB>::BWD_BYTES, st, tq, td, p));
     return 0;
 }
 
 int attn_fwd_wgmma(const AttnParams& p, const AttnDropOffset& off, cudaStream_t st) {
     const int nkb = (p.S + kBlk - 1) / kBlk;
+    VB_REQUIRE(p.drop_scale == 0.f || (reinterpret_cast<uintptr_t>(p.keep) & 15) == 0, "attention: the keep-mask buffer must be 16-byte aligned");
     int rc = attn_keep_mask(p, off, nkb, st);
     if (rc) return rc;
     CUtensorMap tq;
@@ -362,6 +483,7 @@
 
 int attn_bwd_wgmma(const AttnParams& p, cudaStream_t st, bool delta_ready) {
     const int nkb = (p.S + kBlk - 1) / kBlk;
+    VB_REQUIRE(p.drop_scale == 0.f || (reinterpret_cast<uintptr_t>(p.keep) & 15) == 0, "attention: the keep-mask buffer must be 16-byte aligned");
     int rc = 0;
     if (!delta_ready) {
         rc = attn_delta(p, st);
diff --git a/visualbert_b200/csrc/vb_common.cuh b/visualbert_b200/csrc/vb_common.cuh
--- a/visualbert_b200/csrc/vb_common.cuh
+++ b/visualbert_b200/csrc/vb_common.cuh
@@ -230,6 +230,12 @@
         : "memory");
 }
 
+__device__ __forceinline__ void bulk_load(uint32_t smem_dst, const void* src, uint32_t bytes, uint32_t bar) {
+    asm volatile("cp.async.bulk.shared::cluster.global.mbarrier::complete_tx::bytes [%0], [%1], %2, [%3];"
+                 ::"r"(smem_dst), "l"(reinterpret_cast<uint64_t>(src)), "r"(bytes), "r"(bar)
+                 : "memory");
+}
+
 __device__ __forceinline__ uint64_t wgmma_desc_sw128(uint32_t saddr, uint32_t lbo_bytes, uint32_t sbo_bytes) {
     return static_cast<uint64_t>((saddr & 0x3FFFFu) >> 4) | (static_cast<uint64_t>((lbo_bytes >> 4) & 0x3FFFu) << 16) |
            (static_cast<uint64_t>((sbo_bytes >> 4) & 0x3FFFu) << 32) | (1ull << 62);
diff --git a/visualbert_b200/csrc/vb_internal.h b/visualbert_b200/csrc/vb_internal.h
--- a/visualbert_b200/csrc/vb_internal.h
+++ b/visualbert_b200/csrc/vb_internal.h
@@ -18,12 +18,13 @@
              float dropout_p, unsigned long long seed, unsigned stream_id, cudaStream_t st);
 int attn_bwd(const void* qkv, const float* mask_bias, const void* ctx, const float* lse, const void* keep,
              const void* dctx, void* dqkv, float* drow, int B, int S, int A, int H, float dropout_p,
-             unsigned long long seed, unsigned stream_id, cudaStream_t st, bool delta_ready = false);
+             unsigned long long seed, unsigned stream_id, cudaStream_t st, bool delta_ready = false, float* dbias = nullptr);
 int attn_fwd_varlen(const void* qkv, const int* cu_seqlens, void* ctx, float* lse, void* keep, int B, int max_seq, int total,
                     int A, int H, float dropout_p, unsigned long long seed, unsigned stream_id, cudaStream_t st, bool need_lse = true);
 int attn_bwd_varlen(const void* qkv, const int* cu_seqlens, const void* ctx, const float* lse, const void* keep,
                     const void* dctx, void* dqkv, float* drow, int B, int max_seq, int total, int A, int H, float dropout_p,
-                    unsigned long long seed, unsigned stream_id, cudaStream_t st, bool delta_ready = false);
+                    unsigned long long seed, unsigned stream_id, cudaStream_t st, bool delta_ready = false,
+                    float* dbias = nullptr);
 long long attn_keep_bytes(int B, int S, int A);
 int attn_probs(const void* qkv, const float* mask_bias, float* probs, int B, int S, int A, int H, cudaStream_t st);
 int wgrad_splits(long long tiles, int k_blocks);
```

Result: no change. 4338, median of 6 (+0.9%).
